# modal-labs/modal-examples

Measured on AMD Instinct MI355X. Metric: SDXL 1024px images/sec (whole node), higher is better.
Workload: dtype bf16; 1 GPU; model=sdxl-base-unet-2.6b, global_batch=16, image=1024x1024, denoise_steps=4, parallelism=dp1, hipgraph=True

## Files before the change

modal_examples_amd/models/sdxl/layers.py:

```python
from __future__ import annotations

import math

import torch
import torch.nn as nn

from ...ops import functional as OF


class _F32ParamCache:

    def _f32(self, name: str):
        p = getattr(self, name)
        if self.training or p.requires_grad and torch.is_grad_enabled():
            return p.float()
        cache = self.__dict__.setdefault("_f32_cache", {})
        ent = cache.get(name)
        if ent is None or ent[1] is not p or ent[2] != p._version:
            ent = (p.detach().float(), p, p._version)
            cache[name] = ent
        return ent[0]


class LayerNormK(nn.Module, _F32ParamCache):

    def __init__(self, dim: int, eps: float = 1e-5):
        super().__init__()
        self.weight = nn.Parameter(torch.ones(dim))
        self.bias = nn.Parameter(torch.zeros(dim))
        self.eps = eps

    def forward(self, x):
        return OF.layernorm(x, self._f32("weight"), self._f32("bias"), self.eps)


class RMSNormK(nn.Module, _F32ParamCache):
    def __init__(self, dim: int, eps: float = 1e-6):
        super().__init__()
        self.weight = nn.Parameter(torch.ones(dim))
        self.eps = eps

    def forward(self, x):
        return OF.rmsnorm(x, self._f32("weight"), self.eps)


class GroupNormSiLU(nn.Module, _F32ParamCache):

    def __init__(self, channels: int, groups: int = 32, eps: float = 1e-5,
                 silu: bool = True):
        super().__init__()
        self.weight = nn.Parameter(torch.ones(channels))
        self.bias = nn.Parameter(torch.zeros(channels))
        self.groups = groups
        self.eps = eps
        self.silu = silu

    def forward(self, x):
        return OF.groupnorm_silu(x, self._f32("weight"), self._f32("bias"),
                                 self.groups, self.eps, self.silu)


class Conv3x3(nn.Conv2d):

    def __init__(self, c_in: int, c_out: int):
        super().__init__(c_in, c_out, 3, padding=1)

    def _packed(self):
        w, bias = self.weight, self.bias
        bv = None if bias is None else bias._version
        ent = self.__dict__.get("_wr_cache")
        if (ent is None or ent[1] is not w or ent[2] != w._version
                or ent[3] is not bias or ent[4] != bv):
            wr = OF.repack_conv3x3_weight(w.detach())
            b = (bias.detach().float().contiguous() if bias is not None
                 else torch.zeros(w.shape[0], device=w.device))
            ent = ((wr, b), w, w._version, bias, bv)
            self.__dict__["_wr_cache"] = ent
        return ent[0]

    def _use_kernel(self, x) -> bool:
        if not x.is_cuda or x.dtype is not torch.bfloat16 or self.training:
            return False
        if torch.is_grad_enabled() and (x.requires_grad or
                                        self.weight.requires_grad):
            return False
        return True

    def forward_gn(self, x, gn, residual=None, upsample: bool = False):
        if self._use_kernel(x) and gn.silu:
            wr, b = self._packed()
            return OF.conv3x3_gn(x, wr, b, self.out_channels,
                                 gn._f32("weight"), gn._f32("bias"),
                                 gn.groups, gn.eps, residual=residual,
                                 raw_weight=self.weight, upsample=upsample)
        return self.forward(gn(x), residual=residual, upsample=upsample)

    def forward(self, x, residual=None, upsample: bool = False):
        if self._use_kernel(x):
            wr, b = self._packed()
            return OF.conv3x3(x, wr, b, self.out_channels, residual=residual,
                              raw_weight=self.weight, upsample=upsample)
        if upsample:
            x = nn.functional.interpolate(x, scale_factor=2.0, mode="nearest")
        y = nn.functional.conv2d(x, self.weight, self.bias, padding=1)
        return y if residual is None else y + residual


class Conv1x1(nn.Conv2d):

    def __init__(self, c_in: int, c_out: int):
        super().__init__(c_in, c_out, 1)


class SelfAttention(nn.Module):

    def __init__(self, dim: int, head_dim: int = 64):
        super().__init__()
        assert dim % head_dim == 0
        self.heads = dim // head_dim
        self.head_dim = head_dim
        self.qkv = nn.Linear(dim, 3 * dim, bias=False)
        self.out = nn.Linear(dim, dim, bias=True)

    def forward(self, x):
        B, S, C = x.shape
        qkv = self.qkv(x).view(B, S, 3, self.heads, self.head_dim)
        o = OF.attention_qkv(qkv[:, :, 0], qkv[:, :, 1], qkv[:, :, 2])
        return self.out(o)


class CrossAttention(nn.Module):

    def __init__(self, dim: int, ctx_dim: int, head_dim: int = 64):
        super().__init__()
        self.heads = dim // head_dim
        self.head_dim = head_dim
        self.q = nn.Linear(dim, dim, bias=False)
        self.kv = nn.Linear(ctx_dim, 2 * dim, bias=False)
        self.out = nn.Linear(dim, dim, bias=True)

    def forward(self, x, ctx):
        B, S, C = x.shape
        Sk = ctx.shape[1]
        q = self.q(x).view(B, S, self.heads, self.head_dim)
        kv = self.kv(ctx).view(B, Sk, 2, self.heads, self.head_dim)
        o = OF.attention_qkv(q, kv[:, :, 0], kv[:, :, 1])
        return self.out(o)


class GEGLUFeedForward(nn.Module):

    def __init__(self, dim: int, mult: int = 4):
        super().__init__()
        inner = dim * mult
        self.proj_in = nn.Linear(dim, 2 * inner, bias=True)
        self.proj_out = nn.Linear(inner, dim, bias=True)
        self.inner = inner

    def forward(self, x):
        return self.proj_out(OF.glu_fused(self.proj_in(x), gelu=True))


class TransformerBlock(nn.Module):

    def __init__(self, dim: int, ctx_dim: int, head_dim: int = 64):
        super().__init__()
        self.norm1 = LayerNormK(dim)
        self.attn1 = SelfAttention(dim, head_dim)
        self.norm2 = LayerNormK(dim)
        self.attn2 = CrossAttention(dim, ctx_dim, head_dim)
        self.norm3 = LayerNormK(dim)
        self.ff = GEGLUFeedForward(dim)

    def forward(self, x, ctx):
        x = x + self.attn1(self.norm1(x))
        x = x + self.attn2(self.norm2(x), ctx)
        x = x + self.ff(self.norm3(x))
        return x


def timestep_embedding(t: torch.Tensor, dim: int, max_period: float = 10000.0):
    half = dim // 2
    freqs = torch.exp(
        -math.log(max_period) * torch.arange(half, dtype=torch.float32, device=t.device) / half
    )
    args = t.float()[:, None] * freqs[None]
    return torch.cat([torch.cos(args), torch.sin(args)], dim=-1)
```

modal_examples_amd/models/sdxl/unet.py:

```python
from __future__ import annotations

from dataclasses import dataclass

import torch
import torch.nn as nn

from .layers import (
    Conv1x1,
    Conv3x3,
    GroupNormSiLU,
    TransformerBlock,
    timestep_embedding,
)


@dataclass
class UNetConfig:
    in_channels: int = 4
    out_channels: int = 4
    channels: tuple = (320, 640, 1280)
    layers_per_block: int = 2
    transformer_depth: tuple = (0, 2, 10)
    ctx_dim: int = 2048
    head_dim: int = 64
    time_embed_dim: int = 1280
    pooled_dim: int = 1280
    fourier_dim: int = 128
    addition_dim: int = 2816

    @staticmethod
    def sdxl() -> "UNetConfig":
        return UNetConfig()

    @staticmethod
    def small() -> "UNetConfig":
        return UNetConfig(channels=(64, 128, 256), transformer_depth=(0, 1, 2),
                          ctx_dim=256, head_dim=64, time_embed_dim=256,
                          pooled_dim=256, fourier_dim=16,
                          addition_dim=256 + 6 * 32)


class ResnetBlock(nn.Module):
    def __init__(self, c_in: int, c_out: int, temb_dim: int):
        super().__init__()
        self.norm1 = GroupNormSiLU(c_in)
        self.conv1 = Conv3x3(c_in, c_out)
        self.temb_proj = nn.Linear(temb_dim, c_out)
        self.norm2 = GroupNormSiLU(c_out)
        self.conv2 = Conv3x3(c_out, c_out)
        self.skip = Conv1x1(c_in, c_out) if c_in != c_out else nn.Identity()

    def forward(self, x, temb):
        h = self.conv1(self.norm1(x))
        h = h + self.temb_proj(torch.nn.functional.silu(temb))[:, :, None, None]
        return self.conv2(self.norm2(h), residual=self.skip(x))


class SpatialTransformer(nn.Module):

    def __init__(self, channels: int, depth: int, ctx_dim: int, head_dim: int):
        super().__init__()
        self.norm = GroupNormSiLU(channels, silu=False)
        self.proj_in = nn.Linear(channels, channels)
        self.blocks = nn.ModuleList(
            [TransformerBlock(channels, ctx_dim, head_dim) for _ in range(depth)]
        )
        self.proj_out = nn.Linear(channels, channels)

    def forward(self, x, ctx):
        B, C, H, W = x.shape
        res = x
        h = self.norm(x).permute(0, 2, 3, 1).reshape(B, H * W, C)
        h = self.proj_in(h)
        for blk in self.blocks:
            h = blk(h, ctx)
        h = self.proj_out(h)
        return res + h.reshape(B, H, W, C).permute(0, 3, 1, 2)


class Downsample(nn.Module):
    def __init__(self, c):
        super().__init__()
        self.conv = nn.Conv2d(c, c, 3, stride=2, padding=1)

    def forward(self, x):
        return self.conv(x)


class Upsample(nn.Module):
    def __init__(self, c):
        super().__init__()
        self.conv = Conv3x3(c, c)

    def forward(self, x):
        return self.conv(x, upsample=True)


class UNetXL(nn.Module):
    def __init__(self, cfg: UNetConfig = None):
        super().__init__()
        cfg = cfg or UNetConfig.sdxl()
        self.cfg = cfg
        ch = cfg.channels
        ted = cfg.time_embed_dim

        self.conv_in = Conv3x3(cfg.in_channels, ch[0])
        self.time_mlp = nn.Sequential(
            nn.Linear(ch[0], ted), nn.SiLU(), nn.Linear(ted, ted)
        )
        self.add_mlp = nn.Sequential(
            nn.Linear(cfg.addition_dim, ted), nn.SiLU(), nn.Linear(ted, ted)
        )

        self.down_blocks = nn.ModuleList()
        self.downsamplers = nn.ModuleList()
        skip_chs = [ch[0]]
        c_prev = ch[0]
        for lvl, c in enumerate(ch):
            blocks = nn.ModuleList()
            for _ in range(cfg.layers_per_block):
                entry = nn.ModuleDict({"resnet": ResnetBlock(c_prev, c, ted)})
                if cfg.transformer_depth[lvl] > 0:
                    entry["attn"] = SpatialTransformer(
                        c, cfg.transformer_depth[lvl], cfg.ctx_dim, cfg.head_dim
                    )
                blocks.append(entry)
                c_prev = c
                skip_chs.append(c)
            self.down_blocks.append(blocks)
            if lvl < len(ch) - 1:
                self.downsamplers.append(Downsample(c))
                skip_chs.append(c)
            else:
                self.downsamplers.append(nn.Identity())

        top = ch[-1]
        self.mid_res1 = ResnetBlock(top, top, ted)
        self.mid_attn = SpatialTransformer(top, cfg.transformer_depth[-1],
                                           cfg.ctx_dim, cfg.head_dim)
        self.mid_res2 = ResnetBlock(top, top, ted)

        self.up_blocks = nn.ModuleList()
        self.upsamplers = nn.ModuleList()
        c_prev = top
        for lvl in reversed(range(len(ch))):
            c = ch[lvl]
            blocks = nn.ModuleList()
            for _ in range(cfg.layers_per_block + 1):
                skip_c = skip_chs.pop()
                entry = nn.ModuleDict(
                    {"resnet": ResnetBlock(c_prev + skip_c, c, ted)}
                )
                if cfg.transformer_depth[lvl] > 0:
                    entry["attn"] = SpatialTransformer(
                        c, cfg.transformer_depth[lvl], cfg.ctx_dim, cfg.head_dim
                    )
                blocks.append(entry)
                c_prev = c
            self.up_blocks.append(blocks)
            if lvl > 0:
                self.upsamplers.append(Upsample(c))
            else:
                self.upsamplers.append(nn.Identity())

        self.norm_out = GroupNormSiLU(ch[0])
        self.conv_out = Conv3x3(ch[0], cfg.out_channels)

    def forward(self, x, t, ctx, pooled_add):
        dt = x.dtype
        temb = self.time_mlp(timestep_embedding(t, self.cfg.channels[0]).to(dt))
        temb = temb + self.add_mlp(pooled_add)

        h = self.conv_in(x)
        skips = [h]
        for lvl, blocks in enumerate(self.down_blocks):
            for entry in blocks:
                h = entry["resnet"](h, temb)
                if "attn" in entry:
                    h = entry["attn"](h, ctx)
                skips.append(h)
            if not isinstance(self.downsamplers[lvl], nn.Identity):
                h = self.downsamplers[lvl](h)
                skips.append(h)

        h = self.mid_res1(h, temb)
        h = self.mid_attn(h, ctx)
        h = self.mid_res2(h, temb)

        for i, blocks in enumerate(self.up_blocks):
            for entry in blocks:
                h = torch.cat([h, skips.pop()], dim=1)
                h = entry["resnet"](h, temb)
                if "attn" in entry:
                    h = entry["attn"](h, ctx)
            if not isinstance(self.upsamplers[i], nn.Identity):
                h = self.upsamplers[i](h)

        return self.conv_out(self.norm_out(h))
```

modal_examples_amd/models/sdxl/vae.py:

```python
from __future__ import annotations

import torch
import torch.nn as nn

from .layers import Conv1x1, Conv3x3, GroupNormSiLU


class VAEResnet(nn.Module):
    def __init__(self, c_in, c_out):
        super().__init__()
        self.norm1 = GroupNormSiLU(c_in)
        self.conv1 = Conv3x3(c_in, c_out)
        self.norm2 = GroupNormSiLU(c_out)
        self.conv2 = Conv3x3(c_out, c_out)
        self.skip = Conv1x1(c_in, c_out) if c_in != c_out else nn.Identity()

    def forward(self, x):
        h = self.conv1(self.norm1(x))
        return self.conv2(self.norm2(h), residual=self.skip(x))


class VAEMidAttention(nn.Module):

    def __init__(self, c, chunk=2048):
        super().__init__()
        self.norm = GroupNormSiLU(c, silu=False)
        self.q = nn.Linear(c, c)
        self.k = nn.Linear(c, c)
        self.v = nn.Linear(c, c)
        self.out = nn.Linear(c, c)
        self.chunk = chunk
        self.scale = c ** -0.5

    def forward(self, x):
        B, C, H, W = x.shape
        h = self.norm(x).permute(0, 2, 3, 1).reshape(B, H * W, C)
        q, k, v = self.q(h), self.k(h), self.v(h)
        outs = []
        for i in range(0, q.shape[1], self.chunk):
            s = torch.matmul(q[:, i:i + self.chunk], k.transpose(1, 2)) * self.scale
            p = torch.softmax(s.float(), dim=-1).to(v.dtype)
            outs.append(torch.matmul(p, v))
        o = self.out(torch.cat(outs, dim=1))
        return x + o.reshape(B, H, W, C).permute(0, 3, 1, 2)


class VAEDecoder(nn.Module):
    def __init__(self, latent_channels=4, channels=(512, 512, 256, 128),
                 out_channels=3, resnets_per_level=3, scaling_factor=0.13025):
        super().__init__()
        self.scaling_factor = scaling_factor
        c0 = channels[0]
        self.conv_in = Conv3x3(latent_channels, c0)
        self.mid_res1 = VAEResnet(c0, c0)
        self.mid_attn = VAEMidAttention(c0)
        self.mid_res2 = VAEResnet(c0, c0)
        self.levels = nn.ModuleList()
        c_prev = c0
        for li, c in enumerate(channels):
            blocks = nn.ModuleList()
            for _ in range(resnets_per_level):
                blocks.append(VAEResnet(c_prev, c))
                c_prev = c
            up = Conv3x3(c, c) if li < len(channels) - 1 else None
            self.levels.append(nn.ModuleList([blocks, nn.ModuleList([up] if up else [])]))
        self.norm_out = GroupNormSiLU(channels[-1])
        self.conv_out = Conv3x3(channels[-1], out_channels)

    def forward(self, z):
        h = self.conv_in(z / self.scaling_factor)
        h = self.mid_res2(self.mid_attn(self.mid_res1(h)))
        for blocks, ups in self.levels:
            for blk in blocks:
                h = blk(h)
            if len(ups):
                h = ups[0](h, upsample=True)
        return self.conv_out(self.norm_out(h))


class VAEDecoderSmall(VAEDecoder):
    def __init__(self):
        super().__init__(channels=(64, 64, 32, 32))
```

modal_examples_amd/ops/csrc/bindings.cpp:

```cpp
#include <torch/extension.h>
#include <c10/hip/HIPStream.h>
#include <hip/hip_runtime.h>

#include <unordered_map>
#include <vector>

extern "C" {
int fa32_fwd_strided_bf16(const void*, const void*, const void*, void*, float*,
                          int, int, int, int, int, int, float, int,
                          const long long*, hipStream_t);
int fa_bwd_strided_bf16(const void*, const void*, const void*, const void*,
                        const void*, const float*, float*, void*, void*, void*,
                        int, int, int, int, int, int, float, int,
                        const long long*, hipStream_t);
int paged_decode_bf16(const void*, const void*, const void*, const int*,
                      const int*, void*, float*, int, int, int, int, int,
                      int, int, float, int, hipStream_t);
int paged_prefill_bf16(const void*, const void*, const void*, const int*,
                       const int*, const int*, void*, int, int, int, int, int,
                       int, int, float, int, hipStream_t);
void groupnorm_silu_bf16(const void*, void*, float*, const float*,
                         const float*, int, int, long long, int, float, int,
                         hipStream_t);
void layernorm_bf16(const void*, void*, const float*, const float*, long long,
                    int, float, hipStream_t);
void rmsnorm_bf16(const void*, void*, const float*, long long, int, float,
                  hipStream_t);
void cfg_euler_bf16(const void*, const void*, const void*, void*, float, float,
                    long long, hipStream_t);
void silu_mul_bf16(const void*, const void*, void*, long long, hipStream_t);
void geglu_bf16(const void*, const void*, void*, long long, hipStream_t);
void glu_fused_bf16(const void*, void*, long long, long long, int,
                    hipStream_t);
void add_bf16(const void*, const void*, void*, long long, hipStream_t);
void rope_bf16(void*, const float*, const float*, long long, int, int, int,
               long long, long long, long long, const int*, hipStream_t);
void adamw_step(void*, const void*, float*, float*, long long, float, float,
                float, float, float, int, int, hipStream_t);
void gumbel_sample(const float*, unsigned long long*, int*, int, int,
                   float, unsigned long long, hipStream_t);
void sampling_cutoff(const float*, const float*, const int*, const float*,
                     const float*, float*, int, int, hipStream_t);
void gumbel_sample_batch(const float*, const float*, const long long*,
                         const long long*, const float*, unsigned long long*,
                         int*, int, int, hipStream_t);
void softmax_rows(const float*, float*, int, int, hipStream_t);
void scale_in_dev_bf16(const void*, void*, const float*, const long long*,
                       long long, hipStream_t);
void cfg_euler_dev_bf16(const void*, const void*, const void*, void*,
                        const float*, const long long*, float, long long,
                        hipStream_t);
void advance_step(long long*, hipStream_t);
void conv3x3_bf16(const void*, const void*, const void*, const void*, void*,
                  const float*, const float*, int, int, int, int, int, int,
                  int, int, hipStream_t);
void gn_conv_coeffs_bf16(const void*, float*, const float*, const float*,
                         float*, float*, int, int, int, long long, int, float,
                         hipStream_t);
int moe_max_tiles(long long, int, int);
int moe_route_f32(const float*, float*, int*, long long, int, int,
                  hipStream_t);
int moe_ffn_bf16(const void*, const void*, const void*, const float*,
                 const int*, int*, void*, float*, void*, long long, int, int,
                 int, int, hipStream_t);
}

namespace {

hipStream_t cur_stream() {
  return (hipStream_t)c10::hip::getCurrentHIPStream().stream();
}

void check_bf16(const torch::Tensor& t, const char* name) {
  TORCH_CHECK(t.is_cuda(), name, " must be on GPU");
  TORCH_CHECK(t.scalar_type() == torch::kBFloat16, name, " must be bf16");
  TORCH_CHECK(t.is_contiguous(), name, " must be contiguous");
}


void check_bhsd(const torch::Tensor& t, const char* name) {
  TORCH_CHECK(t.is_cuda(), name, " must be on GPU");
  TORCH_CHECK(t.scalar_type() == torch::kBFloat16, name, " must be bf16");
  TORCH_CHECK(t.dim() == 4, name, " must be [B,H,S,D]");
  TORCH_CHECK(t.stride(3) == 1, name, ": head_dim must be contiguous");
}

struct AttnDims {
  int B, Hq, Hkv, Sq, Sk, D;
};

AttnDims check_qkv(const char* op, const torch::Tensor& q,
                   const torch::Tensor& k, const torch::Tensor& v) {
  check_bhsd(q, "q");
  check_bhsd(k, "k");
  check_bhsd(v, "v");
  AttnDims d{(int)q.size(0), (int)q.size(1), (int)k.size(1), (int)q.size(2),
             (int)k.size(2), (int)q.size(3)};
  TORCH_CHECK(d.D == 64 || d.D == 128, op, ": unsupported head_dim ", d.D,
              " (supported: 64, 128)");
  TORCH_CHECK(k.size(0) == d.B && k.size(3) == d.D && v.sizes() == k.sizes(),
              op, ": k/v must be [B,Hkv,Sk,D] matching q's B and D");
  TORCH_CHECK(d.Hkv > 0 && d.Hq % d.Hkv == 0,
              "GQA requires Hq % Hkv == 0, got Hq=", d.Hq, " Hkv=", d.Hkv);
  return d;
}

void push_strides(std::vector<long long>& st, const torch::Tensor& t) {
  st.insert(st.end(), {t.stride(0), t.stride(1), t.stride(2)});
}

std::tuple<torch::Tensor, torch::Tensor> attention_fwd(
    const torch::Tensor& q, const torch::Tensor& k, const torch::Tensor& v,
    bool causal, double scale, bool bshd, bool with_lse,
    const c10::optional<torch::Tensor>& out = c10::nullopt,
    const c10::optional<torch::Tensor>& lse_out = c10::nullopt) {
  const AttnDims d = check_qkv("attention", q, k, v);
  TORCH_CHECK(d.Sk >= 1, "attention: Sk must be at least 1, got Sk=", d.Sk,
              " (a query with no key has no softmax)");
  const std::vector<int64_t> o_shape =
      bshd ? std::vector<int64_t>{d.B, d.Sq, d.Hq, d.D}
           : std::vector<int64_t>{d.B, d.Hq, d.Sq, d.D};
  torch::Tensor o;
  if (out.has_value()) {
    o = *out;
    TORCH_CHECK(o.device() == q.device() && o.scalar_type() == torch::kBFloat16 &&
                o.sizes() == torch::IntArrayRef(o_shape) &&
                (o.numel() == 0 || o.stride(3) == 1),
                "attention: out must be bf16 on the GPU with the output's "
                "shape ", torch::IntArrayRef(o_shape), " and head_dim "
                "contiguous");
  } else {
    o = torch::empty(o_shape, q.options());
  }
  torch::Tensor lse;
  if (with_lse) {
    if (lse_out.has_value()) {
      lse = *lse_out;
      TORCH_CHECK(lse.device() == q.device() && lse.scalar_type() == torch::kFloat32 &&
                  lse.dim() == 3 && lse.size(0) == d.B &&
                  lse.size(1) == d.Hq && lse.size(2) == d.Sq &&
                  lse.is_contiguous(),
                  "attention: lse must be fp32 [B,Hq,Sq] contiguous");
    } else {
      lse = torch::empty({d.B, d.Hq, d.Sq},
                         q.options().dtype(torch::kFloat32));
    }
  }
  if (o.numel() == 0) return {o, lse};
  std::vector<long long> st;
  for (const auto& t : {q, k, v, bshd ? o.transpose(1, 2) : o})
    push_strides(st, t);
  int rc = fa32_fwd_strided_bf16(
      q.data_ptr(), k.data_ptr(), v.data_ptr(), o.data_ptr(),
      with_lse ? lse.data_ptr<float>() : nullptr, d.B, d.Hq, d.Hkv, d.Sq,
      d.Sk, d.D, (float)scale, causal ? 1 : 0, st.data(), cur_stream());
  TORCH_CHECK(rc == 0, "attention: configuration not supported by the kernel "
              "(head_dim must be 64 or 128 and Hq a multiple of Hkv; got D=",
              d.D, " Hq=", d.Hq, " Hkv=", d.Hkv, ")");
  return {o, lse};
}

torch::Tensor attention(torch::Tensor q, torch::Tensor k, torch::Tensor v,
                        bool causal, double scale) {
  check_bf16(q, "q");
  check_bf16(k, "k");
  check_bf16(v, "v");
  return std::get<0>(attention_fwd(q, k, v, causal, scale, false, false));
}

torch::Tensor attention_bshd(torch::Tensor q, torch::Tensor k, torch::Tensor v,
                             bool causal, double scale) {
  return std::get<0>(attention_fwd(q, k, v, causal, scale, true, false));
}

std::tuple<torch::Tensor, torch::Tensor> attention_fwd_lse(
    torch::Tensor q, torch::Tensor k, torch::Tensor v, bool causal,
    double scale, c10::optional<torch::Tensor> out,
    c10::optional<torch::Tensor> lse) {
  return attention_fwd(q, k, v, causal, scale, false, true, out, lse);
}

std::tuple<torch::Tensor, torch::Tensor> attention_fwd_lse_bshd(
    torch::Tensor q, torch::Tensor k, torch::Tensor v, bool causal,
    double scale, c10::optional<torch::Tensor> out,
    c10::optional<torch::Tensor> lse) {
  return attention_fwd(q, k, v, causal, scale, true, true, out, lse);
}

torch::Tensor paged_decode(torch::Tensor q, torch::Tensor kc, torch::Tensor vc,
                           c10::optional<torch::Tensor> block_table,
                           torch::Tensor seq_lens, int64_t block_size,
                           double scale) {
  check_bf16(q, "q");
  const bool kv_fp8 = kc.scalar_type() == torch::kFloat8_e4m3fn;
  TORCH_CHECK(kv_fp8 || kc.scalar_type() == torch::kBFloat16,
              "k_cache must be bf16 or float8_e4m3fn");
  TORCH_CHECK(vc.scalar_type() == kc.scalar_type(), "kv cache dtype mismatch");
  TORCH_CHECK(kc.is_contiguous() && vc.is_contiguous());
  TORCH_CHECK(q.dim() == 3 && kc.dim() == 4, "q must be [B,Hq,D], k_cache "
              "[blocks,Hkv,block_size,D] or [B,Hkv,S,D]");
  int B = q.size(0), Hq = q.size(1), D = q.size(2);
  int Hkv = kc.size(1), max_blocks = 0;
  TORCH_CHECK(D == 64 || D == 128, "paged_decode: unsupported head_dim ", D,
              " (supported: 64, 128)");
  TORCH_CHECK(kc.size(3) == D, "paged_decode: k_cache head_dim ", kc.size(3),
              " != q head_dim ", D);
  TORCH_CHECK(Hkv > 0 && Hq % Hkv == 0, "GQA requires Hq % Hkv == 0, got Hq=",
              Hq, " Hkv=", Hkv);
  TORCH_CHECK(Hq / Hkv <= 8, "paged_decode: unsupported GQA group Hq/Hkv = ",
              Hq / Hkv, " (supported: 1..8)");
  const int* bt_ptr = nullptr;
  if (block_table.has_value()) {
    max_blocks = block_table->size(1);
    bt_ptr = block_table->data_ptr<int>();
  } else {
    block_size = kc.size(2);
  }
  auto o = torch::empty_like(q);
  long long s_bound = block_table.has_value()
      ? (long long)max_blocks * block_size : (long long)kc.size(2);
  int splits = 1;
  while (B * Hkv * splits < 512 && (long long)splits * 128 < s_bound &&
         splits < 64)
    splits *= 2;
  torch::Tensor ws;
  float* ws_ptr = nullptr;
  if (splits > 1) {
    ws = torch::empty({(long long)B * Hq * splits * (D + 2)},
                      q.options().dtype(torch::kFloat32));
    ws_ptr = ws.data_ptr<float>();
  }
  int rc = paged_decode_bf16(q.data_ptr(), kc.data_ptr(), vc.data_ptr(),
                             bt_ptr, seq_lens.data_ptr<int>(), o.data_ptr(),
                             ws_ptr, B, Hq, Hkv, D, (int)block_size,
                             max_blocks, splits, (float)scale, kv_fp8 ? 1 : 0,
                             cur_stream());
  TORCH_CHECK(rc == 0, "paged_decode: configuration not supported by the "
              "kernel (head_dim must be 64 or 128, Hq a multiple of Hkv and "
              "Hq/Hkv in 1..8; got D=", D, " Hq=", Hq, " Hkv=", Hkv, ")");
  return o;
}

torch::Tensor paged_prefill(torch::Tensor q, torch::Tensor kc, torch::Tensor vc,
                            torch::Tensor block_table, torch::Tensor cu_q,
                            torch::Tensor seq_lens, int64_t block_size,
                            double scale, int64_t max_q_len) {
  check_bf16(q, "q");
  TORCH_CHECK(q.dim() == 3, "paged_prefill: q must be [T,Hq,D]");
  const bool kv_fp8 = kc.scalar_type() == torch::kFloat8_e4m3fn;
  TORCH_CHECK(kv_fp8 || kc.scalar_type() == torch::kBFloat16,
              "k_cache must be bf16 or float8_e4m3fn");
  TORCH_CHECK(vc.scalar_type() == kc.scalar_type(), "kv cache dtype mismatch");
  TORCH_CHECK(kc.dim() == 4 && vc.sizes() == kc.sizes() &&
                  kc.is_contiguous() && vc.is_contiguous(),
              "paged_prefill: k_cache/v_cache must be contiguous "
              "[blocks,Hkv,block_size,D] of one shape");
  const int64_t T = q.size(0);
  const int Hq = q.size(1), D = q.size(2), Hkv = kc.size(1);
  TORCH_CHECK(D == 64 || D == 128, "paged_prefill: unsupported head_dim ", D,
              " (supported: 64, 128)");
  TORCH_CHECK(kc.size(3) == D, "paged_prefill: k_cache head_dim ", kc.size(3),
              " != q head_dim ", D);
  TORCH_CHECK(Hkv > 0 && Hq % Hkv == 0, "GQA requires Hq % Hkv == 0, got Hq=",
              Hq, " Hkv=", Hkv);
  TORCH_CHECK(block_size > 0 && kc.size(2) == block_size,
              "paged_prefill: block_size must be positive and the cache's "
              "third dim, got block_size=", block_size, " cache ", kc.sizes());
  TORCH_CHECK(seq_lens.scalar_type() == torch::kInt32 && seq_lens.dim() == 1 &&
                  seq_lens.is_contiguous(),
              "paged_prefill: seq_lens must be int32 [B] contiguous");
  const int64_t B = seq_lens.size(0);
  TORCH_CHECK(block_table.scalar_type() == torch::kInt32 &&
                  block_table.dim() == 2 && block_table.size(0) == B &&
                  block_table.is_contiguous(),
              "paged_prefill: block_table must be int32 [B=", B,
              ", max_blocks] contiguous, got ", block_table.sizes());
  TORCH_CHECK(cu_q.scalar_type() == torch::kInt32 && cu_q.dim() == 1 &&
                  cu_q.size(0) == B + 1 && cu_q.is_contiguous(),
              "paged_prefill: cu_q must be int32 [B+1=", B + 1, "], got ",
              cu_q.sizes());
  for (const torch::Tensor* t : {&kc, &vc, &block_table, &cu_q, &seq_lens})
    TORCH_CHECK(t->device() == q.device(),
                "paged_prefill: all tensors must be on q's device");
  auto o = torch::empty_like(q);
  if (T == 0) return o;
  TORCH_CHECK(max_q_len >= 1, "paged_prefill: max_q_len must be at least 1, "
              "got ", max_q_len);
  TORCH_CHECK(B >= 1, "paged_prefill: ", T, " query rows but no sequence");
  max_q_len = std::min<int64_t>(max_q_len, T);
  int rc = paged_prefill_bf16(
      q.data_ptr(), kc.data_ptr(), vc.data_ptr(), block_table.data_ptr<int>(),
      cu_q.data_ptr<int>(), seq_lens.data_ptr<int>(), o.data_ptr(), (int)B, Hq,
      Hkv, D, (int)block_size, (int)block_table.size(1), (int)max_q_len,
      (float)scale, kv_fp8 ? 1 : 0, cur_stream());
  TORCH_CHECK(rc == 0, "paged_prefill: configuration not supported by the "
              "kernel (head_dim must be 64 or 128, Hq a multiple of Hkv, B "
              "and Hq at most 65535; got D=", D, " Hq=", Hq, " Hkv=", Hkv,
              " B=", B, ")");
  return o;
}

void attention_bwd(torch::Tensor q, torch::Tensor k, torch::Tensor v,
                   torch::Tensor o, torch::Tensor lse, torch::Tensor dout,
                   torch::Tensor dq, torch::Tensor dk, torch::Tensor dv,
                   bool causal, double scale) {
  const AttnDims d = check_qkv("attention_bwd", q, k, v);
  const int B = d.B, Hq = d.Hq, Hkv = d.Hkv, Sq = d.Sq, Sk = d.Sk, D = d.D;
  check_bhsd(o, "o");
  check_bhsd(dout, "dout");
  check_bhsd(dq, "dq");
  check_bhsd(dk, "dk");
  check_bhsd(dv, "dv");
  TORCH_CHECK(B >= 1 && Sq >= 1 && Sk >= 1, "attention_bwd: empty input");
  TORCH_CHECK(o.sizes() == q.sizes() && dout.sizes() == q.sizes(),
              "attention_bwd: o and dout must have q's shape");
  TORCH_CHECK(dq.sizes() == q.sizes() && dk.sizes() == k.sizes() &&
              dv.sizes() == v.sizes(),
              "attention_bwd: dq/dk/dv must have the shapes of q/k/v");
  TORCH_CHECK(lse.is_cuda() && lse.scalar_type() == torch::kFloat32 &&
              lse.dim() == 3 && lse.size(0) == B && lse.size(1) == Hq &&
              lse.size(2) == Sq && lse.is_contiguous(),
              "attention_bwd: lse must be fp32 [B,Hq,Sq] contiguous");
  TORCH_CHECK(!causal || Sk >= Sq, "attention_bwd: causal requires Sk >= Sq, "
              "got Sq=", Sq, " Sk=", Sk);
  auto delta = torch::empty_like(lse);
  std::vector<long long> st;
  for (const auto& t : {q, k, v, o, dout, dq, dk, dv}) push_strides(st, t);
  int rc = fa_bwd_strided_bf16(
      q.data_ptr(), k.data_ptr(), v.data_ptr(), o.data_ptr(), dout.data_ptr(),
      lse.data_ptr<float>(), delta.data_ptr<float>(), dq.data_ptr(),
      dk.data_ptr(), dv.data_ptr(), B, Hq, Hkv, Sq, Sk, D, (float)scale,
      causal ? 1 : 0, st.data(), cur_stream());
  TORCH_CHECK(rc == 0, "attention_bwd: configuration not supported by the "
              "kernel (got D=", D, " Hq=", Hq, " Hkv=", Hkv, " Sq=", Sq,
              " Sk=", Sk, " causal=", causal, ")");
}


torch::Tensor groupnorm_silu(torch::Tensor x, torch::Tensor gamma,
                             torch::Tensor beta, int64_t groups, double eps,
                             bool do_silu) {
  check_bf16(x, "x");
  TORCH_CHECK(x.dim() == 4, "x must be NCHW");
  int N = x.size(0), C = x.size(1);
  long long HW = (long long)x.size(2) * x.size(3);
  auto y = torch::empty_like(x);
  auto ws = torch::zeros({N * groups * 2},
                         x.options().dtype(torch::kFloat32));
  groupnorm_silu_bf16(x.data_ptr(), y.data_ptr(), ws.data_ptr<float>(),
                      gamma.data_ptr<float>(), beta.data_ptr<float>(), N, C,
                      HW, (int)groups, (float)eps, do_silu ? 1 : 0,
                      cur_stream());
  return y;
}

torch::Tensor layernorm(torch::Tensor x, torch::Tensor gamma,
                        torch::Tensor beta, double eps) {
  check_bf16(x, "x");
  int D = x.size(-1);
  long long rows = x.numel() / D;
  auto y = torch::empty_like(x);
  layernorm_bf16(x.data_ptr(), y.data_ptr(), gamma.data_ptr<float>(),
                 beta.data_ptr<float>(), rows, D, (float)eps, cur_stream());
  return y;
}

torch::Tensor rmsnorm(torch::Tensor x, torch::Tensor gamma, double eps) {
  check_bf16(x, "x");
  int D = x.size(-1);
  TORCH_CHECK(D % 8 == 0, "rmsnorm needs D % 8 == 0");
  long long rows = x.numel() / D;
  auto y = torch::empty_like(x);
  rmsnorm_bf16(x.data_ptr(), y.data_ptr(), gamma.data_ptr<float>(), rows, D,
               (float)eps, cur_stream());
  return y;
}


torch::Tensor cfg_euler(torch::Tensor xt, torch::Tensor eps_c,
                        c10::optional<torch::Tensor> eps_u, double guidance,
                        double dsigma) {
  check_bf16(xt, "x_t");
  auto xn = torch::empty_like(xt);
  cfg_euler_bf16(xt.data_ptr(), eps_c.data_ptr(),
                 eps_u.has_value() ? eps_u->data_ptr() : nullptr,
                 xn.data_ptr(), (float)guidance, (float)dsigma, xt.numel(),
                 cur_stream());
  return xn;
}

torch::Tensor silu_mul(torch::Tensor a, torch::Tensor b) {
  check_bf16(a, "a");
  auto y = torch::empty_like(a);
  silu_mul_bf16(a.data_ptr(), b.data_ptr(), y.data_ptr(), a.numel(),
                cur_stream());
  return y;
}

torch::Tensor geglu(torch::Tensor a, torch::Tensor b) {
  check_bf16(a, "a");
  auto y = torch::empty_like(a);
  geglu_bf16(a.data_ptr(), b.data_ptr(), y.data_ptr(), a.numel(), cur_stream());
  return y;
}

torch::Tensor glu_fused(torch::Tensor src, bool gelu) {
  check_bf16(src, "src");
  long long inner = src.size(-1) / 2;
  TORCH_CHECK(src.size(-1) % 2 == 0 && inner % 8 == 0,
              "inner dim must be even and 8-aligned");
  long long rows = src.numel() / (2 * inner);
  auto sizes = src.sizes().vec();
  sizes.back() = inner;
  auto y = torch::empty(sizes, src.options());
  glu_fused_bf16(src.data_ptr(), y.data_ptr(), rows, inner, gelu ? 1 : 0,
                 cur_stream());
  return y;
}

torch::Tensor add_residual(torch::Tensor a, torch::Tensor b) {
  check_bf16(a, "a");
  auto y = torch::empty_like(a);
  add_bf16(a.data_ptr(), b.data_ptr(), y.data_ptr(), a.numel(), cur_stream());
  return y;
}

void rope_(torch::Tensor qk, torch::Tensor cosv, torch::Tensor sinv,
           c10::optional<torch::Tensor> positions) {
  TORCH_CHECK(qk.is_cuda() && qk.scalar_type() == torch::kBFloat16);
  TORCH_CHECK(qk.dim() == 4 && qk.stride(3) == 1,
              "qk must be [B,H,S,D] with contiguous head_dim");
  long long B = qk.size(0);
  int H = qk.size(1), S = qk.size(2), D = qk.size(3);
  if (positions.has_value())
    TORCH_CHECK(positions->numel() == B * S || positions->numel() == S,
                "positions must be [B*S] (or [S] with B==1)");
  rope_bf16(qk.data_ptr(), cosv.data_ptr<float>(), sinv.data_ptr<float>(), B,
            H, S, D, qk.stride(0), qk.stride(1), qk.stride(2),
            positions.has_value() ? positions->data_ptr<int>() : nullptr,
            cur_stream());
}

void adamw_(torch::Tensor p, torch::Tensor g, torch::Tensor m, torch::Tensor v,
            double lr, double beta1, double beta2, double eps, double wd,
            int64_t step) {
  TORCH_CHECK(p.is_cuda() && p.is_contiguous(), "p must be contiguous GPU");
  bool bf16 = p.scalar_type() == torch::kBFloat16;
  adamw_step(p.data_ptr(), g.data_ptr(), m.data_ptr<float>(),
             v.data_ptr<float>(), p.numel(), (float)lr, (float)beta1,
             (float)beta2, (float)eps, (float)wd, (int)step, bf16 ? 1 : 0,
             cur_stream());
}


void check_f32_vec(const torch::Tensor& t, const char* name, int64_t n,
                   const char* len) {
  TORCH_CHECK(t.is_cuda(), name, " must be on GPU");
  TORCH_CHECK(t.scalar_type() == torch::kFloat, name, " must be fp32");
  TORCH_CHECK(t.is_contiguous(), name, " must be contiguous");
  TORCH_CHECK(t.numel() == n, name, " must have ", len, " = ", n,
              " elements, got ", t.numel());
}

struct ConvDims {
  int N, C, H, W, Ho, Wo, Kpad, C16;
};

ConvDims check_conv(const char* op, const torch::Tensor& x,
                    const torch::Tensor& wr, const torch::Tensor& bias,
                    const c10::optional<torch::Tensor>& residual, int64_t K,
                    bool upsample) {
  check_bf16(x, "x");
  check_bf16(wr, "wr");
  TORCH_CHECK(x.dim() == 4, op, ": x must be NCHW, got ", x.dim(), " dims");
  TORCH_CHECK(wr.dim() == 3 && wr.size(0) == 9 && wr.size(1) > 0 &&
                  wr.size(2) > 0 && wr.size(1) % 64 == 0 &&
                  wr.size(2) % 16 == 0,
              op, ": wr must be [9, Kpad, C16] (repacked 3x3 weights) with "
              "Kpad % 64 == 0 and C16 % 16 == 0, got ", wr.sizes());
  ConvDims d{(int)x.size(0), (int)x.size(1), (int)x.size(2), (int)x.size(3),
             0, 0, (int)wr.size(1), (int)wr.size(2)};
  d.Ho = upsample ? d.H * 2 : d.H;
  d.Wo = upsample ? d.W * 2 : d.W;
  TORCH_CHECK(K >= 1, op, ": K must be at least 1, got ", K);
  TORCH_CHECK(K <= d.Kpad && d.C <= d.C16, op,
              ": weight pack smaller than conv (K=", K, " > Kpad=", d.Kpad,
              " or C=", d.C, " > C16=", d.C16, ")");
  TORCH_CHECK((int64_t)d.C16 * d.H * d.W < (1ll << 30) &&
                  64ll * d.Ho * d.Wo < (1ll << 31) &&
                  9ll * d.Kpad * d.C16 < (1ll << 31),
              op, ": too large for the kernel's 32-bit offsets (C16*H*W must "
              "stay below 2^30, 64*Ho*Wo and 9*Kpad*C16 below 2^31), got x ",
              x.sizes(), " wr ", wr.sizes());
  check_f32_vec(bias, "bias", K, "K");
  if (residual.has_value()) {
    check_bf16(*residual, "residual");
    TORCH_CHECK(residual->dim() == 4 && residual->size(0) == d.N &&
                    residual->size(1) == K && residual->size(2) == d.Ho &&
                    residual->size(3) == d.Wo,
                op, ": residual shape mismatch: ", residual->sizes(),
                " against output [", d.N, ", ", K, ", ", d.Ho, ", ", d.Wo, "]");
  }
  return d;
}

torch::Tensor conv3x3(torch::Tensor x, torch::Tensor wr, torch::Tensor bias,
                      c10::optional<torch::Tensor> residual, int64_t K,
                      bool upsample) {
  const ConvDims d = check_conv("conv3x3", x, wr, bias, residual, K, upsample);
  auto out = torch::empty({d.N, K, d.Ho, d.Wo}, x.options());
  conv3x3_bf16(x.data_ptr(), wr.data_ptr(), bias.data_ptr(),
               residual.has_value() ? residual->data_ptr() : nullptr,
               out.data_ptr(), nullptr, nullptr, d.N, d.C, d.Ho, d.Wo, (int)K,
               d.C16, d.Kpad, upsample ? 1 : 0, cur_stream());
  return out;
}

torch::Tensor conv3x3_gn(torch::Tensor x, torch::Tensor wr, torch::Tensor bias,
                         c10::optional<torch::Tensor> residual, int64_t K,
                         bool upsample, torch::Tensor gamma,
                         torch::Tensor beta, int64_t groups, double eps) {
  const ConvDims d =
      check_conv("conv3x3_gn", x, wr, bias, residual, K, upsample);
  check_f32_vec(gamma, "gamma", d.C, "C");
  check_f32_vec(beta, "beta", d.C, "C");
  TORCH_CHECK(groups >= 1 && d.C % groups == 0,
              "conv3x3_gn: groups must be at least 1 and divide C, got groups=",
              groups, " C=", d.C);
  const int N = d.N, C16 = d.C16;
  long long HW = (long long)d.H * d.W;
  auto fopt = x.options().dtype(torch::kFloat32);
  auto ws = torch::zeros({(long long)N * groups * 2}, fopt);
  auto scale = torch::empty({(long long)N * C16}, fopt);
  auto shift = torch::empty({(long long)N * C16}, fopt);
  gn_conv_coeffs_bf16(x.data_ptr(), ws.data_ptr<float>(),
                      gamma.data_ptr<float>(), beta.data_ptr<float>(),
                      scale.data_ptr<float>(), shift.data_ptr<float>(), N, d.C,
                      C16, HW, (int)groups, (float)eps, cur_stream());
  auto out = torch::empty({N, K, d.Ho, d.Wo}, x.options());
  conv3x3_bf16(x.data_ptr(), wr.data_ptr(), bias.data_ptr(),
               residual.has_value() ? residual->data_ptr() : nullptr,
               out.data_ptr(), scale.data_ptr<float>(),
               shift.data_ptr<float>(), N, d.C, d.Ho, d.Wo, (int)K, C16,
               d.Kpad, upsample ? 1 : 0, cur_stream());
  return out;
}


std::tuple<torch::Tensor, torch::Tensor> moe_route(torch::Tensor logits,
                                                   int64_t top_k) {
  TORCH_CHECK(logits.is_cuda() && logits.scalar_type() == torch::kFloat32 &&
                  logits.dim() == 2 && logits.is_contiguous(),
              "moe_route: logits must be fp32 [N,E] contiguous on GPU");
  const int64_t N = logits.size(0), E = logits.size(1);
  TORCH_CHECK(N >= 1, "moe_route: logits has no rows");
  TORCH_CHECK(E >= 1 && E <= 128, "moe_route: logits has E=", E,
              " experts (supported: 1..128)");
  TORCH_CHECK(top_k >= 1 && top_k <= 8 && top_k <= E, "moe_route: top_k=",
              top_k, " (supported: 1..min(E, 8), E=", E, ")");
  auto w = torch::empty({N, top_k}, logits.options());
  auto idx = torch::empty({N, top_k}, logits.options().dtype(torch::kInt32));
  int rc = moe_route_f32(logits.data_ptr<float>(), w.data_ptr<float>(),
                         idx.data_ptr<int>(), N, (int)E, (int)top_k,
                         cur_stream());
  TORCH_CHECK(rc == 0, "moe_route: logits shape ", logits.sizes(),
              " with top_k=", top_k, " not supported by the kernel");
  return {w, idx};
}

torch::Tensor moe_ffn(torch::Tensor x, torch::Tensor gate_up,
                      torch::Tensor down, torch::Tensor weights,
                      torch::Tensor idx) {
  check_bf16(x, "x");
  check_bf16(gate_up, "gate_up");
  check_bf16(down, "down");
  TORCH_CHECK(x.dim() == 2 && gate_up.dim() == 3 && down.dim() == 3,
              "moe_ffn: x must be [N,dim], gate_up [E,2*ffn_dim,dim], down "
              "[E,dim,ffn_dim]");
  const int64_t N = x.size(0), d = x.size(1), E = gate_up.size(0),
                F = down.size(2);
  TORCH_CHECK(N >= 1, "moe_ffn: x has no rows");
  TORCH_CHECK(d >= 64 && d % 64 == 0, "moe_ffn: x has dim=", d,
              " (must be a multiple of 64)");
  TORCH_CHECK(F >= 64 && F % 64 == 0, "moe_ffn: down has ffn_dim=", F,
              " (must be a multiple of 64)");
  TORCH_CHECK(E >= 1 && E <= 128, "moe_ffn: gate_up has E=", E,
              " experts (supported: 1..128)");
  TORCH_CHECK(gate_up.size(1) == 2 * F && gate_up.size(2) == d &&
                  down.size(0) == E && down.size(1) == d,
              "moe_ffn: gate_up ", gate_up.sizes(), " / down ", down.sizes(),
              " do not match [E,2*ffn_dim,dim] / [E,dim,ffn_dim] with dim=",
              d);
  TORCH_CHECK(idx.is_cuda() && idx.scalar_type() == torch::kInt32 &&
                  idx.dim() == 2 && idx.size(0) == N && idx.is_contiguous(),
              "moe_ffn: idx must be int32 [N,top_k] contiguous on GPU");
  const int64_t k = idx.size(1);
  TORCH_CHECK(k >= 1 && k <= 8 && k <= E, "moe_ffn: idx has top_k=", k,
              " (supported: 1..min(E, 8), E=", E, ")");
  TORCH_CHECK(weights.is_cuda() && weights.scalar_type() == torch::kFloat32 &&
                  weights.sizes() == idx.sizes() && weights.is_contiguous(),
              "moe_ffn: weights must be fp32 [N,top_k] contiguous on GPU");
  for (const torch::Tensor* t : {&gate_up, &down, &weights, &idx})
    TORCH_CHECK(t->device() == x.device(),
                "moe_ffn: all tensors must be on x's device");
  TORCH_CHECK(N * k < (1ll << 30) && N * k * d < (1ll << 40),
              "moe_ffn: x has too many rows (N=", N, ")");
  const int64_t tiles = moe_max_tiles(N, (int)k, (int)E);
  auto iopt = x.options().dtype(torch::kInt32);
  auto sched = torch::empty({tiles * 32 + tiles + 1}, iopt);
  auto h = torch::empty({tiles * 32, F}, x.options());
  auto y = torch::empty({N * k, d}, x.options().dtype(torch::kFloat32));
  auto out = torch::empty({N, d}, x.options());
  int rc = moe_ffn_bf16(x.data_ptr(), gate_up.data_ptr(), down.data_ptr(),
                        weights.data_ptr<float>(), idx.data_ptr<int>(),
                        sched.data_ptr<int>(), h.data_ptr(),
                        y.data_ptr<float>(), out.data_ptr(), N, (int)d,
                        (int)F, (int)E, (int)k, cur_stream());
  TORCH_CHECK(rc == 0, "moe_ffn: shape not supported by the kernel (N=", N,
              " dim=", d, " ffn_dim=", F, " E=", E, " top_k=", k, ")");
  return out;
}

torch::Tensor sample_gumbel(torch::Tensor logits, double temperature,
                            int64_t seed) {
  TORCH_CHECK(logits.is_cuda() && logits.scalar_type() == torch::kFloat32,
              "logits must be f32 GPU");
  int rows = logits.size(0), V = logits.size(1);
  auto out = torch::empty({rows}, logits.options().dtype(torch::kInt32));
  auto keys = torch::zeros({rows}, logits.options().dtype(torch::kInt64));
  gumbel_sample(logits.data_ptr<float>(),
                (unsigned long long*)keys.data_ptr<int64_t>(),
                out.data_ptr<int>(), rows, V, (float)temperature,
                (unsigned long long)seed, cur_stream());
  return out;
}


void check_logits2d(const torch::Tensor& logits) {
  TORCH_CHECK(logits.is_cuda() && logits.scalar_type() == torch::kFloat32,
              "logits must be f32 GPU");
  TORCH_CHECK(logits.dim() == 2 && logits.is_contiguous(),
              "logits must be [rows, V] contiguous");
  TORCH_CHECK(logits.size(0) > 0 && logits.size(1) > 0 &&
              logits.size(1) < (1ll << 31) && logits.size(0) < (1ll << 22),
              "logits: unsupported shape ", logits.sizes());
}

void check_row_param(const torch::Tensor& t, const torch::Tensor& logits,
                     torch::ScalarType dt, const char* name) {
  TORCH_CHECK(t.is_cuda() && t.device() == logits.device(), name,
              " must be on the logits' GPU");
  TORCH_CHECK(t.scalar_type() == dt, name, " must be ", dt);
  TORCH_CHECK(t.dim() == 1 && t.size(0) == logits.size(0), name,
              " must have one value per row ([", logits.size(0), "]), got ",
              t.sizes());
  TORCH_CHECK(t.is_contiguous(), name, " must be contiguous");
}

torch::Tensor sampling_cutoff_fwd(torch::Tensor logits, torch::Tensor temps,
                                  torch::Tensor top_k, torch::Tensor top_p,
                                  torch::Tensor min_p) {
  check_logits2d(logits);
  check_row_param(temps, logits, torch::kFloat32, "temperature");
  check_row_param(top_k, logits, torch::kInt32, "top_k");
  check_row_param(top_p, logits, torch::kFloat32, "top_p");
  check_row_param(min_p, logits, torch::kFloat32, "min_p");
  int rows = logits.size(0), V = logits.size(1);
  auto cut = torch::empty({rows}, logits.options());
  sampling_cutoff(logits.data_ptr<float>(), temps.data_ptr<float>(),
                  top_k.data_ptr<int>(), top_p.data_ptr<float>(),
                  min_p.data_ptr<float>(), cut.data_ptr<float>(), rows, V,
                  cur_stream());
  return cut;
}

torch::Tensor sample_batch(torch::Tensor logits, torch::Tensor temps,
                           torch::Tensor seeds, torch::Tensor counters,
                           c10::optional<torch::Tensor> cutoff) {
  check_logits2d(logits);
  check_row_param(temps, logits, torch::kFloat32, "temperature");
  check_row_param(seeds, logits, torch::kInt64, "seeds");
  check_row_param(counters, logits, torch::kInt64, "counters");
  if (cutoff.has_value())
    check_row_param(*cutoff, logits, torch::kFloat32, "cutoff");
  int rows = logits.size(0), V = logits.size(1);
  auto out = torch::empty({rows}, logits.options().dtype(torch::kInt32));
  auto keys = torch::zeros({rows}, logits.options().dtype(torch::kInt64));
  gumbel_sample_batch(
      logits.data_ptr<float>(), temps.data_ptr<float>(),
      (const long long*)seeds.data_ptr<int64_t>(),
      (const long long*)counters.data_ptr<int64_t>(),
      cutoff.has_value() ? cutoff->data_ptr<float>() : nullptr,
      (unsigned long long*)keys.data_ptr<int64_t>(), out.data_ptr<int>(),
      rows, V, cur_stream());
  return out;
}

torch::Tensor softmax_fwd(torch::Tensor x) {
  TORCH_CHECK(x.is_cuda() && x.scalar_type() == torch::kFloat32);
  int V = x.size(-1);
  long long rows = x.numel() / V;
  auto y = torch::empty_like(x);
  softmax_rows(x.data_ptr<float>(), y.data_ptr<float>(), (int)rows, V,
               cur_stream());
  return y;
}

void scale_in_dev(torch::Tensor x, torch::Tensor y, torch::Tensor sigmas,
                  torch::Tensor step) {
  scale_in_dev_bf16(x.data_ptr(), y.data_ptr(), sigmas.data_ptr<float>(),
                    (const long long*)step.data_ptr<int64_t>(), x.numel(), cur_stream());
}

void cfg_euler_dev(torch::Tensor xt, torch::Tensor eps_c,
                   c10::optional<torch::Tensor> eps_u, torch::Tensor xn,
                   torch::Tensor sigmas, torch::Tensor step, double guidance) {
  cfg_euler_dev_bf16(xt.data_ptr(), eps_c.data_ptr(),
                     eps_u.has_value() ? eps_u->data_ptr() : nullptr,
                     xn.data_ptr(), sigmas.data_ptr<float>(),
                     (const long long*)step.data_ptr<int64_t>(), (float)guidance, xt.numel(),
                     cur_stream());
}

void step_advance(torch::Tensor step) {
  advance_step((long long*)step.data_ptr<int64_t>(), cur_stream());
}


struct SnapRegion {
  void* host = nullptr;
  size_t bytes = 0;
  std::vector<hipStream_t> streams;
  size_t rr = 0;
};

std::unordered_map<int64_t, SnapRegion> g_snaps;
int64_t g_next_snap = 1;

int64_t snap_create(int64_t bytes) {
  SnapRegion r;
  r.bytes = (size_t)bytes;
  TORCH_CHECK(hipHostMalloc(&r.host, r.bytes, hipHostMallocDefault) == hipSuccess,
              "hipHostMalloc failed for ", bytes, " bytes");
  r.streams.resize(4);
  for (auto& s : r.streams)
    TORCH_CHECK(hipStreamCreateWithFlags(&s, hipStreamNonBlocking) == hipSuccess);
  int64_t id = g_next_snap++;
  g_snaps[id] = r;
  return id;
}

void snap_save(int64_t id, int64_t offset, torch::Tensor t) {
  auto& r = g_snaps.at(id);
  size_t n = t.numel() * t.element_size();
  TORCH_CHECK((size_t)offset + n <= r.bytes, "snapshot overflow");
  hipStream_t s = r.streams[r.rr++ % r.streams.size()];
  TORCH_CHECK(hipMemcpyAsync((char*)r.host + offset, t.data_ptr(), n,
                             hipMemcpyDeviceToHost, s) == hipSuccess);
}

void snap_restore(int64_t id, int64_t offset, torch::Tensor t) {
  auto& r = g_snaps.at(id);
  size_t n = t.numel() * t.element_size();
  TORCH_CHECK((size_t)offset + n <= r.bytes, "snapshot overflow");
  hipStream_t s = r.streams[r.rr++ % r.streams.size()];
  TORCH_CHECK(hipMemcpyAsync(t.data_ptr(), (char*)r.host + offset, n,
                             hipMemcpyHostToDevice, s) == hipSuccess);
}

void snap_sync(int64_t id) {
  auto& r = g_snaps.at(id);
  for (auto& s : r.streams) TORCH_CHECK(hipStreamSynchronize(s) == hipSuccess);
}

void snap_free(int64_t id) {
  auto it = g_snaps.find(id);
  if (it == g_snaps.end()) return;
  for (auto& s : it->second.streams) hipStreamDestroy(s);
  hipHostFree(it->second.host);
  g_snaps.erase(it);
}

}

PYBIND11_MODULE(TORCH_EXTENSION_NAME, m) {
  m.def("attention", &attention, "flash attention fwd bf16 (K1/K5/K7)");
  m.def("attention_bshd", &attention_bshd, "stride-aware attention, BSHD out");
  m.def("attention_fwd_lse", &attention_fwd_lse,
        "attention fwd returning (o, lse) for the backward; out= / lse= "
        "write into the caller's tensors",
        py::arg("q"), py::arg("k"), py::arg("v"), py::arg("causal"),
        py::arg("scale"), py::arg("out") = py::none(),
        py::arg("lse") = py::none());
  m.def("attention_fwd_lse_bshd", &attention_fwd_lse_bshd,
        "attention fwd returning (o [B,S,H,D], lse); out= / lse= write into "
        "the caller's tensors",
        py::arg("q"), py::arg("k"), py::arg("v"), py::arg("causal"),
        py::arg("scale"), py::arg("out") = py::none(),
        py::arg("lse") = py::none());
  m.def("attention_bwd", &attention_bwd,
        "flash attention bwd bf16 into caller-provided dq/dk/dv");
  m.def("paged_decode", &paged_decode, "paged KV decode attention (K6)");
  m.def("paged_prefill", &paged_prefill,
        "paged KV prefill attention: ragged causal chunks over a cached "
        "prefix (K6)");
  m.def("groupnorm_silu", &groupnorm_silu);
  m.def("layernorm", &layernorm);
  m.def("rmsnorm", &rmsnorm);
  m.def("cfg_euler", &cfg_euler, "fused CFG + Euler step (K4)");
  m.def("silu_mul", &silu_mul);
  m.def("geglu", &geglu);
  m.def("glu_fused", &glu_fused, "in-place-sliced silu/gelu-mul over a fused [.,2I] projection");
  m.def("add_residual", &add_residual);
  m.def("rope_", &rope_, "in-place RoPE with host cos/sin tables");
  m.def("adamw_", &adamw_, "fused AdamW step (K9)");
  m.def("sample_gumbel", &sample_gumbel, "fused sampling (K8)");
  m.def("sample_batch", &sample_batch,
        "per-row temperature/seed/counter/cutoff gumbel sampling (K8)");
  m.def("sampling_cutoff", &sampling_cutoff_fwd,
        "per-row top-k/top-p/min-p logit cutoff by radix select (K8)");
  m.def("conv3x3", &conv3x3, "NCHW implicit-GEMM 3x3 conv, fused bias+res (K3)");
  m.def("conv3x3_gn", &conv3x3_gn, "GroupNorm+SiLU fused into the K3 conv");
  m.def("softmax_fwd", &softmax_fwd);
  m.def("moe_route", &moe_route,
        "MoE top-k routing: (weights fp32 [N,k], idx int32 [N,k])");
  m.def("moe_ffn", &moe_ffn,
        "fused MoE FFN: on-device schedule, grouped MFMA GEMMs, combine");
  m.def("scale_in_dev", &scale_in_dev, "x * 1/sqrt(sigma^2+1), device sigma");
  m.def("cfg_euler_dev", &cfg_euler_dev, "graph-capturable CFG+Euler step");
  m.def("step_advance", &step_advance, "increment device step counter");
  m.def("snap_create", &snap_create, "pinned-host snapshot region (K13)");
  m.def("snap_save", &snap_save);
  m.def("snap_restore", &snap_restore);
  m.def("snap_sync", &snap_sync);
  m.def("snap_free", &snap_free);
}
```

modal_examples_amd/ops/csrc/conv3x3.hip:

```cpp
#include "common.h"

#include <cstdio>
#include <cstdlib>
#include <type_traits>

#define CV_NW 4
#define CV_COLS 32
#define CV_BK 64
#define CV_CC 16

typedef __attribute__((ext_vector_type(16))) float f32x16c;

DEV_INLINE unsigned gn_silu_bf16(unsigned raw, float sc, float sh) {
  float f = bf2f((short)raw) * sc + sh;
  f = f / (1.f + __expf(-f));
  return (unsigned)(unsigned short)f2bf(f);
}

DEV_INLINE int to_sgpr(int v) {
  int s;
  asm volatile("s_nop 0\n\tv_readfirstlane_b32 %0, %1" : "=s"(s) : "v"(v));
  return s;
}

#define PATCH_C (CV_COLS + 2)

#define WLDS_ELEMS (9 * CV_BK * CV_CC)
#define WSLOTS (WLDS_ELEMS / 8)
#define WSLOTS_PER_T ((WSLOTS + CV_NW * WAVE - 1) / (CV_NW * WAVE))

template <bool UP, bool GN, int RPW>
__global__ __launch_bounds__(CV_NW * WAVE, RPW == 2 ? 3 : 1)
void conv3x3_kernel(
    const short* __restrict__ in, const short* __restrict__ wr,
    const float* __restrict__ bias, const short* __restrict__ res,
    short* __restrict__ out, const float* __restrict__ gn_scale,
    const float* __restrict__ gn_shift, int C, int H, int W, int Hs, int Ws,
    int K, int C16, int Kpad, int npix_x, int npix, int nk) {
  constexpr int CV_ROWS = CV_NW * RPW;
  constexpr int PATCH_R = CV_ROWS + 2;
  constexpr int PATCH_ELEMS = PATCH_R * PATCH_C * CV_CC;
  constexpr int STAGE_SLOTS = PATCH_R * PATCH_C * 2;
  constexpr int SLOTS_PER_T =
      (STAGE_SLOTS + CV_NW * WAVE - 1) / (CV_NW * WAVE);
  __shared__ alignas(16) short patch[PATCH_ELEMS];
  __shared__ alignas(16) short wlds[WLDS_ELEMS];
  __shared__ alignas(16) float bias_s[CV_BK];

  const int tid = threadIdx.x;
  const int w = tid / WAVE;
  const int l = tid % WAVE;
  const int l31 = l & 31;
  const int hi5 = l >> 5;
  const int n = blockIdx.y;

  int bid = blockIdx.x;
  {
    int nwg = npix * nk;
    int q = nwg >> 3, r = nwg & 7;
    int xcd = bid & 7, pos = bid >> 3;
    bid = (xcd < r ? xcd * (q + 1) : r * (q + 1) + (xcd - r) * q) + pos;
  }
  const int ktile = to_sgpr(bid / npix);
  const int pix = bid - ktile * npix;
  const int pix_y = pix / npix_x;
  const int y0 = pix_y * CV_ROWS;
  const int x0 = (pix - pix_y * npix_x) * CV_COLS;
  const int k0 = ktile * CV_BK;

  const long long in_n = (long long)n * C * Hs * Ws;
  const int nc = C16 / CV_CC;

  if (tid < CV_BK) bias_s[tid] = bias[min(k0 + tid, K - 1)];

  const char* in_img = (const char*)(in + in_n);
  const unsigned hwb = (unsigned)Hs * (unsigned)Ws * 2u;
  unsigned soff[SLOTS_PER_T], soff_max[SLOTS_PER_T];
  int slds[SLOTS_PER_T], smask[SLOTS_PER_T];
#pragma unroll
  for (int i = 0; i < SLOTS_PER_T; ++i) {
    const int s_raw = i * CV_NW * WAVE + tid;
    const int s = min(s_raw, STAGE_SLOTS - 1);
    const int col = s % PATCH_C;
    const int u = s / PATCH_C;
    const int oct = u & 1;
    const int row = u >> 1;
    const int y = y0 + row - 1;
    const int x = x0 + col - 1;
    const bool live =
        s_raw < STAGE_SLOTS && y >= 0 && y < H && x >= 0 && x < W;
    const int yc = min(max(y, 0), H - 1);
    const int xc = min(max(x, 0), W - 1);
    const unsigned sy = UP ? (yc >> 1) : yc;
    const unsigned sx = UP ? (xc >> 1) : xc;
    const unsigned pix = (sy * (unsigned)Ws + sx) * 2u;
    soff[i] = pix + (unsigned)(oct * 8) * hwb;
    soff_max[i] = pix + (unsigned)(C - 1) * hwb;
    slds[i] = (row * PATCH_C + col) * CV_CC + oct * 8;
    int m = live ? -1 : 0;
    asm volatile("" : "+v"(m));
    smask[i] = m;
  }

  unsigned sraw[SLOTS_PER_T][8];
  float gsc[GN ? CV_CC : 1], gsh[GN ? CV_CC : 1];
  auto stage_load = [&](int cc) {
#pragma unroll
    for (int i = 0; i < SLOTS_PER_T; ++i) {
#pragma unroll
      for (int j = 0; j < 8; ++j) {
        const unsigned o = min(soff[i] + (unsigned)j * hwb, soff_max[i]);
        sraw[i][j] = *(const unsigned short*)(in_img + o);
      }
      soff[i] += CV_CC * hwb;
    }
    if constexpr (GN) {
      const float* ps = gn_scale + (long long)n * C16 + cc * CV_CC;
      const float* ph = gn_shift + (long long)n * C16 + cc * CV_CC;
#pragma unroll
      for (int j = 0; j < CV_CC; ++j) {
        gsc[j] = ps[j];
        gsh[j] = ph[j];
      }
    }
  };
  auto stage_write = [&](int cc) {
    const int nv = C - cc * CV_CC;
#pragma unroll
    for (int i = 0; i < SLOTS_PER_T; ++i) {
      const int o8 = slds[i] & 8;
      i32x4 pk;
#pragma unroll
      for (int d = 0; d < 4; ++d) {
        unsigned lo = sraw[i][2 * d], hi = sraw[i][2 * d + 1];
        asm volatile("" : "+v"(lo), "+v"(hi));
        if constexpr (GN) {
          lo = gn_silu_bf16(lo, o8 ? gsc[8 + 2 * d] : gsc[2 * d],
                            o8 ? gsh[8 + 2 * d] : gsh[2 * d]);
          hi = gn_silu_bf16(hi, o8 ? gsc[9 + 2 * d] : gsc[1 + 2 * d],
                            o8 ? gsh[9 + 2 * d] : gsh[1 + 2 * d]);
        }
        pk[d] = (int)((lo | (hi << 16)) & (unsigned)smask[i]);
      }
      if (nv < CV_CC) {
        const int nvl = nv - o8;
#pragma unroll
        for (int d = 0; d < 4; ++d) {
          const unsigned lo = (unsigned)((2 * d - nvl) >> 31);
          const unsigned hi = (unsigned)((2 * d + 1 - nvl) >> 31);
          pk[d] &= (int)((lo & 0xffffu) | (hi & 0xffff0000u));
        }
      }
      if ((i + 1) * CV_NW * WAVE <= STAGE_SLOTS ||
          i * CV_NW * WAVE + tid < STAGE_SLOTS)
        *(i32x4*)&patch[slds[i]] = pk;
    }
  };

  bf16x8 wreg[WSLOTS_PER_T];
  unsigned woff[WSLOTS_PER_T];
#pragma unroll
  for (int i = 0; i < WSLOTS_PER_T; ++i) {
    const int s = min(i * CV_NW * WAVE + tid, WSLOTS - 1);
    const int oct = s & 1;
    const int kr = (s >> 1) & (CV_BK - 1);
    const int tap = (s >> 1) >> 6;
    woff[i] = ((unsigned)(tap * Kpad + kr) * (unsigned)C16 + oct * 8) * 2u;
  }
  const char* w_tile = (const char*)(wr + (long long)k0 * C16);
  auto wstage_load = [&](int cc) {
    const char* wb = w_tile + cc * (CV_CC * 2);
#pragma unroll
    for (int i = 0; i < WSLOTS_PER_T; ++i)
      wreg[i] = *(const bf16x8*)(wb + woff[i]);
  };
  auto wstage_write = [&]() {
#pragma unroll
    for (int i = 0; i < WSLOTS_PER_T; ++i) {
      const int s = i * CV_NW * WAVE + tid;
      if ((i + 1) * CV_NW * WAVE <= WSLOTS || s < WSLOTS)
        *(bf16x8*)&wlds[s * 8] = wreg[i];
    }
  };

  f32x16c acc[RPW][2];
#pragma unroll
  for (int a = 0; a < RPW; ++a)
#pragma unroll
    for (int b = 0; b < 2; ++b)
#pragma unroll
      for (int r = 0; r < 16; ++r) acc[a][b][r] = 0.f;

  stage_load(0);
  wstage_load(0);
  for (int cc = 0; cc < nc; ++cc) {
    __syncthreads();
    stage_write(cc);
    wstage_write();
    __syncthreads();
    if (cc + 1 < nc) {
      stage_load(cc + 1);
      wstage_load(cc + 1);
    }

    const short* wl = &wlds[l31 * CV_CC + hi5 * 8];
    const short* pl = &patch[(w * RPW * PATCH_C + l31) * CV_CC + hi5 * 8];
#pragma unroll
    for (int tap = 0; tap < 9; ++tap) {
      const int dy = tap / 3, dx = tap - 3 * (tap / 3);
      bf16x8 a0 = *(const bf16x8*)&wl[tap * CV_BK * CV_CC];
      bf16x8 a1 = *(const bf16x8*)&wl[(tap * CV_BK + 32) * CV_CC];
#pragma unroll
      for (int rr = 0; rr < RPW; ++rr) {
        bf16x8 b =
            *(const bf16x8*)&pl[((rr + dy) * PATCH_C + dx) * CV_CC];
        __builtin_amdgcn_s_setprio(1);
        acc[rr][0] = __builtin_amdgcn_mfma_f32_32x32x16_bf16(a0, b, acc[rr][0], 0, 0, 0);
        acc[rr][1] = __builtin_amdgcn_mfma_f32_32x32x16_bf16(a1, b, acc[rr][1], 0, 0, 0);
        __builtin_amdgcn_s_setprio(0);
      }
    }
  }

  auto epilogue = [&](auto res_c, auto edge_c) {
    constexpr bool RES = decltype(res_c)::value;
    constexpr bool EDGE = decltype(edge_c)::value;
    int t = tid;
    asm volatile("" : "+v"(t));
    const int w = t / WAVE, l31 = t & 31, hi5 = (t >> 5) & 1;
    const unsigned hw = (unsigned)H * (unsigned)W;
    const long long slab = ((long long)n * K + k0) * hw;
    const char* resb = RES ? (const char*)(res + slab) : nullptr;
    char* outb = (char*)(out + slab);
    const int x = x0 + l31;
    const int kmax = K - 1 - k0;
#pragma unroll
    for (int rr = 0; rr < RPW; ++rr) {
      const int y = y0 + w * RPW + rr;
      const bool pix_ok = !EDGE || (y < H && x < W);
      const unsigned po = EDGE ? (unsigned)min(y, H - 1) * W + min(x, W - 1)
                               : (unsigned)y * W + x;
#pragma unroll
      for (int mf = 0; mf < 2; ++mf) {
        unsigned rv[16];
        if constexpr (RES) {
#pragma unroll
          for (int r = 0; r < 16; ++r) {
            const int kl = mf * 32 + (r & 3) + 8 * (r >> 2) + 4 * hi5;
            const unsigned ke = EDGE ? min(kl, kmax) : kl;
            rv[r] = *(const unsigned short*)(resb + (po + ke * hw) * 2u);
          }
        }
#pragma unroll
        for (int q = 0; q < 4; ++q) {
          const f32x4 b4 = *(const f32x4*)&bias_s[mf * 32 + 8 * q + 4 * hi5];
#pragma unroll
          for (int j = 0; j < 4; ++j) {
            const int r = q * 4 + j;
            const int kl = mf * 32 + j + 8 * q + 4 * hi5;
            float v = acc[rr][mf][r] + b4[j];
            if constexpr (RES) v += bf2f((short)rv[r]);
            if (!EDGE || (pix_ok && kl <= kmax))
              *(short*)(outb + (po + (unsigned)kl * hw) * 2u) = f2bf(v);
          }
        }
      }
    }
  };
  const bool edge =
      y0 + CV_ROWS > H || x0 + CV_COLS > W || k0 + CV_BK > K;
  if (res != nullptr) {
    if (edge) epilogue(std::true_type{}, std::true_type{});
    else epilogue(std::true_type{}, std::false_type{});
  } else {
    if (edge) epilogue(std::false_type{}, std::true_type{});
    else epilogue(std::false_type{}, std::false_type{});
  }
}

extern "C" void conv3x3_bf16(const void* in, const void* wrepack,
                             const void* bias, const void* residual, void* out,
                             const float* gn_scale, const float* gn_shift,
                             int N, int C, int H, int W, int K, int C16,
                             int Kpad, int upsample, hipStream_t stream) {
  const int Hs = upsample ? H / 2 : H;
  const int Ws = upsample ? W / 2 : W;
  static const int rpw = [] {
    const char* e = getenv("MODAL_AMD_CONV_RPW");
    return (e && atoi(e) == 4) ? 4 : 2;
  }();
  const int rows = CV_NW * rpw;
  const int npix_x = (W + CV_COLS - 1) / CV_COLS;
  const int npix_y = (H + rows - 1) / rows;
  const int npix = npix_x * npix_y;
  const int nk = (K + CV_BK - 1) / CV_BK;
  dim3 grid(npix * nk, N);
  dim3 block(CV_NW * WAVE);
  const bool gn = gn_scale != nullptr;
#define CVL(UPV, GNV, RPWV) \
  hipLaunchKernelGGL((conv3x3_kernel<UPV, GNV, RPWV>), grid, block, 0, \
                     stream, (const short*)in, (const short*)wrepack, \
                     (const float*)bias, (const short*)residual, (short*)out, \
                     gn_scale, gn_shift, C, H, W, Hs, Ws, K, C16, Kpad, \
                     npix_x, npix, nk)
  if (rpw == 4) {
    if (upsample) {
      if (gn) CVL(true, true, 4); else CVL(true, false, 4);
    } else {
      if (gn) CVL(false, true, 4); else CVL(false, false, 4);
    }
  } else {
    if (upsample) {
      if (gn) CVL(true, true, 2); else CVL(true, false, 2);
    } else {
      if (gn) CVL(false, true, 2); else CVL(false, false, 2);
    }
  }
#undef CVL
}
```

modal_examples_amd/ops/csrc/elementwise.hip:

```cpp
#include "common.h"

#define EW_BLOCK 256


__global__ __launch_bounds__(EW_BLOCK) void cfg_euler_kernel(
    const short* __restrict__ Xt, const short* __restrict__ EpsC,
    const short* __restrict__ EpsU, short* __restrict__ Xn, float guidance,
    float dsigma, long long n) {
  long long stride = (long long)gridDim.x * EW_BLOCK * 8;
  for (long long i = ((long long)blockIdx.x * EW_BLOCK + threadIdx.x) * 8;
       i + 8 <= n; i += stride) {
    bf16x8 x = *(const bf16x8*)&Xt[i];
    bf16x8 ec = *(const bf16x8*)&EpsC[i];
    bf16x8 o;
    if (EpsU != nullptr) {
      bf16x8 eu = *(const bf16x8*)&EpsU[i];
#pragma unroll
      for (int j = 0; j < 8; ++j) {
        float e = bf2f(eu[j]) + guidance * (bf2f(ec[j]) - bf2f(eu[j]));
        o[j] = f2bf(bf2f(x[j]) + dsigma * e);
      }
    } else {
#pragma unroll
      for (int j = 0; j < 8; ++j)
        o[j] = f2bf(bf2f(x[j]) + dsigma * bf2f(ec[j]));
    }
    *(bf16x8*)&Xn[i] = o;
  }
  long long full = (n / 8) * 8;
  for (long long i = full + (long long)blockIdx.x * EW_BLOCK + threadIdx.x;
       i < n; i += (long long)gridDim.x * EW_BLOCK) {
    float e = bf2f(EpsC[i]);
    if (EpsU != nullptr) {
      float eu = bf2f(EpsU[i]);
      e = eu + guidance * (e - eu);
    }
    Xn[i] = f2bf(bf2f(Xt[i]) + dsigma * e);
  }
}

extern "C" void cfg_euler_bf16(const void* xt, const void* eps_c,
                               const void* eps_u, void* xn, float guidance,
                               float dsigma, long long n, hipStream_t stream) {
  int grid = elementwise_grid(n, EW_BLOCK);
  hipLaunchKernelGGL(cfg_euler_kernel, dim3(grid), dim3(EW_BLOCK), 0, stream,
                     (const short*)xt, (const short*)eps_c,
                     (const short*)eps_u, (short*)xn, guidance, dsigma, n);
}


__global__ __launch_bounds__(EW_BLOCK) void silu_mul_kernel(
    const short* __restrict__ A, const short* __restrict__ Bv,
    short* __restrict__ Y, long long n) {
  long long stride = (long long)gridDim.x * EW_BLOCK * 8;
  for (long long i = ((long long)blockIdx.x * EW_BLOCK + threadIdx.x) * 8;
       i + 8 <= n; i += stride) {
    bf16x8 a = *(const bf16x8*)&A[i];
    bf16x8 b = *(const bf16x8*)&Bv[i];
    bf16x8 o;
#pragma unroll
    for (int j = 0; j < 8; ++j) {
      float f = bf2f(a[j]);
      o[j] = f2bf(f / (1.f + __expf(-f)) * bf2f(b[j]));
    }
    *(bf16x8*)&Y[i] = o;
  }
  long long full = (n / 8) * 8;
  for (long long i = full + (long long)blockIdx.x * EW_BLOCK + threadIdx.x;
       i < n; i += (long long)gridDim.x * EW_BLOCK) {
    float f = bf2f(A[i]);
    Y[i] = f2bf(f / (1.f + __expf(-f)) * bf2f(Bv[i]));
  }
}

extern "C" void silu_mul_bf16(const void* a, const void* b, void* y,
                              long long n, hipStream_t stream) {
  int grid = elementwise_grid(n, EW_BLOCK);
  hipLaunchKernelGGL(silu_mul_kernel, dim3(grid), dim3(EW_BLOCK), 0, stream,
                     (const short*)a, (const short*)b, (short*)y, n);
}


__global__ __launch_bounds__(EW_BLOCK) void geglu_kernel(
    const short* __restrict__ A, const short* __restrict__ Bv,
    short* __restrict__ Y, long long n) {
  long long stride = (long long)gridDim.x * EW_BLOCK * 8;
  const float k0 = 0.7978845608028654f, k1 = 0.044715f;
  for (long long i = ((long long)blockIdx.x * EW_BLOCK + threadIdx.x) * 8;
       i + 8 <= n; i += stride) {
    bf16x8 a = *(const bf16x8*)&A[i];
    bf16x8 b = *(const bf16x8*)&Bv[i];
    bf16x8 o;
#pragma unroll
    for (int j = 0; j < 8; ++j) {
      float f = bf2f(a[j]);
      float g = 0.5f * f * (1.f + tanhf(k0 * (f + k1 * f * f * f)));
      o[j] = f2bf(g * bf2f(b[j]));
    }
    *(bf16x8*)&Y[i] = o;
  }
  long long full = (n / 8) * 8;
  for (long long i = full + (long long)blockIdx.x * EW_BLOCK + threadIdx.x;
       i < n; i += (long long)gridDim.x * EW_BLOCK) {
    float f = bf2f(A[i]);
    float g = 0.5f * f * (1.f + tanhf(k0 * (f + k1 * f * f * f)));
    Y[i] = f2bf(g * bf2f(Bv[i]));
  }
}

extern "C" void geglu_bf16(const void* a, const void* b, void* y, long long n,
                           hipStream_t stream) {
  int grid = elementwise_grid(n, EW_BLOCK);
  hipLaunchKernelGGL(geglu_kernel, dim3(grid), dim3(EW_BLOCK), 0, stream,
                     (const short*)a, (const short*)b, (short*)y, n);
}


__global__ __launch_bounds__(EW_BLOCK) void add_kernel(
    const short* __restrict__ A, const short* __restrict__ Bv,
    short* __restrict__ Y, long long n) {
  long long stride = (long long)gridDim.x * EW_BLOCK * 8;
  for (long long i = ((long long)blockIdx.x * EW_BLOCK + threadIdx.x) * 8;
       i + 8 <= n; i += stride) {
    bf16x8 a = *(const bf16x8*)&A[i];
    bf16x8 b = *(const bf16x8*)&Bv[i];
    bf16x8 o;
#pragma unroll
    for (int j = 0; j < 8; ++j) o[j] = f2bf(bf2f(a[j]) + bf2f(b[j]));
    *(bf16x8*)&Y[i] = o;
  }
  long long full = (n / 8) * 8;
  for (long long i = full + (long long)blockIdx.x * EW_BLOCK + threadIdx.x;
       i < n; i += (long long)gridDim.x * EW_BLOCK)
    Y[i] = f2bf(bf2f(A[i]) + bf2f(Bv[i]));
}

extern "C" void add_bf16(const void* a, const void* b, void* y, long long n,
                         hipStream_t stream) {
  int grid = elementwise_grid(n, EW_BLOCK);
  hipLaunchKernelGGL(add_kernel, dim3(grid), dim3(EW_BLOCK), 0, stream,
                     (const short*)a, (const short*)b, (short*)y, n);
}


__global__ __launch_bounds__(EW_BLOCK) void rope_kernel(
    short* __restrict__ Qk, const float* __restrict__ Cos,
    const float* __restrict__ Sin, long long B, int H, int S, int D,
    long long bst, long long hst, long long sst,
    const int* __restrict__ positions ) {
  long long rows = B * H * S;
  int l = threadIdx.x % WAVE;
  for (long long row = blockIdx.x * (EW_BLOCK / WAVE) + threadIdx.x / WAVE;
       row < rows; row += (long long)gridDim.x * (EW_BLOCK / WAVE)) {
    int s = (int)(row % S);
    int h = (int)((row / S) % H);
    long long b = row / ((long long)H * S);
    int pos = positions != nullptr ? positions[b * S + s] : s;
    short* x = Qk + b * bst + h * hst + s * sst;
    for (int i = l * 2; i < D / 2; i += WAVE * 2) {
      float c0 = Cos[(long long)pos * (D / 2) + i];
      float s0 = Sin[(long long)pos * (D / 2) + i];
      float c1 = Cos[(long long)pos * (D / 2) + i + 1];
      float s1 = Sin[(long long)pos * (D / 2) + i + 1];
      float x0 = bf2f(x[i]), x2 = bf2f(x[i + D / 2]);
      float x1 = bf2f(x[i + 1]), x3 = bf2f(x[i + 1 + D / 2]);
      x[i] = f2bf(x0 * c0 - x2 * s0);
      x[i + D / 2] = f2bf(x2 * c0 + x0 * s0);
      x[i + 1] = f2bf(x1 * c1 - x3 * s1);
      x[i + 1 + D / 2] = f2bf(x3 * c1 + x1 * s1);
    }
  }
}

extern "C" void rope_bf16(void* qk, const float* cosv, const float* sinv,
                          long long B, int H, int S, int D, long long bst,
                          long long hst, long long sst, const int* positions,
                          hipStream_t stream) {
  long long rows = B * (long long)H * S;
  int grid = (int)((rows + 3) / 4);
  if (grid > 4096) grid = 4096;
  hipLaunchKernelGGL(rope_kernel, dim3(grid), dim3(EW_BLOCK), 0, stream,
                     (short*)qk, cosv, sinv, B, H, S, D, bst, hst, sst,
                     positions);
}


__global__ __launch_bounds__(EW_BLOCK) void scale_in_dev_kernel(
    const short* __restrict__ X, short* __restrict__ Y,
    const float* __restrict__ sigmas, const long long* __restrict__ step,
    long long n) {
  float s = sigmas[(int)*step];
  float c = rsqrtf(s * s + 1.f);
  long long stride = (long long)gridDim.x * EW_BLOCK * 8;
  for (long long i = ((long long)blockIdx.x * EW_BLOCK + threadIdx.x) * 8;
       i + 8 <= n; i += stride) {
    bf16x8 x = *(const bf16x8*)&X[i];
    bf16x8 o;
#pragma unroll
    for (int j = 0; j < 8; ++j) o[j] = f2bf(bf2f(x[j]) * c);
    *(bf16x8*)&Y[i] = o;
  }
  long long full = (n / 8) * 8;
  for (long long i = full + (long long)blockIdx.x * EW_BLOCK + threadIdx.x;
       i < n; i += (long long)gridDim.x * EW_BLOCK)
    Y[i] = f2bf(bf2f(X[i]) * c);
}

__global__ __launch_bounds__(EW_BLOCK) void cfg_euler_dev_kernel(
    const short* __restrict__ Xt, const short* __restrict__ EpsC,
    const short* __restrict__ EpsU, short* __restrict__ Xn,
    const float* __restrict__ sigmas, const long long* __restrict__ step,
    float guidance, long long n) {
  int st = (int)*step;
  float dsigma = sigmas[st + 1] - sigmas[st];
  long long stride = (long long)gridDim.x * EW_BLOCK * 8;
  for (long long i = ((long long)blockIdx.x * EW_BLOCK + threadIdx.x) * 8;
       i + 8 <= n; i += stride) {
    bf16x8 x = *(const bf16x8*)&Xt[i];
    bf16x8 ec = *(const bf16x8*)&EpsC[i];
    bf16x8 o;
    if (EpsU != nullptr) {
      bf16x8 eu = *(const bf16x8*)&EpsU[i];
#pragma unroll
      for (int j = 0; j < 8; ++j) {
        float e = bf2f(eu[j]) + guidance * (bf2f(ec[j]) - bf2f(eu[j]));
        o[j] = f2bf(bf2f(x[j]) + dsigma * e);
      }
    } else {
#pragma unroll
      for (int j = 0; j < 8; ++j)
        o[j] = f2bf(bf2f(x[j]) + dsigma * bf2f(ec[j]));
    }
    *(bf16x8*)&Xn[i] = o;
  }
  long long full = (n / 8) * 8;
  for (long long i = full + (long long)blockIdx.x * EW_BLOCK + threadIdx.x;
       i < n; i += (long long)gridDim.x * EW_BLOCK) {
    float e = bf2f(EpsC[i]);
    if (EpsU != nullptr) {
      float eu = bf2f(EpsU[i]);
      e = eu + guidance * (e - eu);
    }
    Xn[i] = f2bf(bf2f(Xt[i]) + dsigma * e);
  }
}

__global__ void advance_step_kernel(long long* step) {
  if (threadIdx.x == 0 && blockIdx.x == 0) *step += 1;
}

extern "C" void scale_in_dev_bf16(const void* x, void* y, const float* sigmas,
                                  const long long* step, long long n,
                                  hipStream_t stream) {
  int grid = elementwise_grid(n, EW_BLOCK);
  hipLaunchKernelGGL(scale_in_dev_kernel, dim3(grid), dim3(EW_BLOCK), 0,
                     stream, (const short*)x, (short*)y, sigmas, step, n);
}

extern "C" void cfg_euler_dev_bf16(const void* xt, const void* eps_c,
                                   const void* eps_u, void* xn,
                                   const float* sigmas, const long long* step,
                                   float guidance, long long n,
                                   hipStream_t stream) {
  int grid = elementwise_grid(n, EW_BLOCK);
  hipLaunchKernelGGL(cfg_euler_dev_kernel, dim3(grid), dim3(EW_BLOCK), 0,
                     stream, (const short*)xt, (const short*)eps_c,
                     (const short*)eps_u, (short*)xn, sigmas, step, guidance,
                     n);
}

extern "C" void advance_step(long long* step, hipStream_t stream) {
  hipLaunchKernelGGL(advance_step_kernel, dim3(1), dim3(64), 0, stream, step);
}


template <bool GELU>
__global__ __launch_bounds__(EW_BLOCK) void glu_fused_kernel(
    const short* __restrict__ Src, short* __restrict__ Y, long long rows,
    long long inner) {
  const float k0 = 0.7978845608028654f, k1 = 0.044715f;
  long long n = rows * inner;
  long long stride = (long long)gridDim.x * EW_BLOCK * 8;
  for (long long i = ((long long)blockIdx.x * EW_BLOCK + threadIdx.x) * 8;
       i + 8 <= n; i += stride) {
    long long row = i / inner, c = i - row * inner;
    const short* base = Src + row * 2 * inner + c;
    bf16x8 a = *(const bf16x8*)base;
    bf16x8 b = *(const bf16x8*)(base + inner);
    bf16x8 o;
#pragma unroll
    for (int j = 0; j < 8; ++j) {
      float f = bf2f(a[j]);
      float act;
      if (GELU) {
        float t = tanhf(k0 * (f + k1 * f * f * f));
        act = 0.5f * f * (1.f + t);
      } else {
        act = f / (1.f + __expf(-f));
      }
      o[j] = f2bf(act * bf2f(b[j]));
    }
    *(bf16x8*)&Y[i] = o;
  }
  long long full = (n / 8) * 8;
  for (long long i = full + (long long)blockIdx.x * EW_BLOCK + threadIdx.x;
       i < n; i += (long long)gridDim.x * EW_BLOCK) {
    long long row = i / inner, c = i - row * inner;
    float f = bf2f(Src[row * 2 * inner + c]);
    float bb = bf2f(Src[row * 2 * inner + inner + c]);
    float act;
    if (GELU) {
      float t = tanhf(k0 * (f + k1 * f * f * f));
      act = 0.5f * f * (1.f + t);
    } else {
      act = f / (1.f + __expf(-f));
    }
    Y[i] = f2bf(act * bb);
  }
}

extern "C" void glu_fused_bf16(const void* src, void* y, long long rows,
                               long long inner, int gelu,
                               hipStream_t stream) {
  int grid = elementwise_grid(rows * inner, EW_BLOCK);
  if (gelu)
    hipLaunchKernelGGL((glu_fused_kernel<true>), dim3(grid), dim3(EW_BLOCK),
                       0, stream, (const short*)src, (short*)y, rows, inner);
  else
    hipLaunchKernelGGL((glu_fused_kernel<false>), dim3(grid), dim3(EW_BLOCK),
                       0, stream, (const short*)src, (short*)y, rows, inner);
}
```

modal_examples_amd/ops/csrc/norms.hip:

```cpp
#include "common.h"


__global__ __launch_bounds__(256) void gn_partial_kernel(
    const short* __restrict__ X, float* __restrict__ WS, int N, int C,
    long long HW, int G, int split) {
  const int blk = blockIdx.x;
  const int ng = blk / split;
  const int sp = blk % split;
  const int n = ng / G, g = ng % G;
  const int cpg = C / G;
  const short* x = X + ((long long)n * C + (long long)g * cpg) * HW;
  long long per = (((HW + split - 1) / split) + 7) & ~7LL;
  long long lo = sp * per, hi = min(HW, lo + per);
  if (lo >= HW) return;
  float s = 0.f, ss = 0.f;
  for (int c = 0; c < cpg; ++c) {
    const short* xc = x + (long long)c * HW;
    long long i = lo + (long long)threadIdx.x * 8;
    for (; i + 8 <= hi; i += 256 * 8) {
      bf16x8 v = *(const bf16x8*)&xc[i];
#pragma unroll
      for (int j = 0; j < 8; ++j) {
        float f = bf2f(v[j]);
        s += f;
        ss += f * f;
      }
    }
    long long tail = hi - ((hi - lo) % 8);
    for (long long t = tail + threadIdx.x; t < hi; t += 256) {
      if (t >= lo) {
        float f = bf2f(xc[t]);
        s += f;
        ss += f * f;
      }
    }
  }
  s = wave_sum(s);
  ss = wave_sum(ss);
  if ((threadIdx.x & (WAVE - 1)) == 0) {
    atomicAdd(&WS[ng * 2], s);
    atomicAdd(&WS[ng * 2 + 1], ss);
  }
}

__global__ __launch_bounds__(256) void gn_norm_kernel(
    const short* __restrict__ X, short* __restrict__ Y,
    const float* __restrict__ WS, const float* __restrict__ gamma,
    const float* __restrict__ beta, int N, int C, long long HW, int G,
    float eps, int do_silu, int split) {
  const int blk = blockIdx.x;
  const int ng = blk / split;
  const int sp = blk % split;
  const int n = ng / G, g = ng % G;
  const int cpg = C / G;
  const long long slab = (long long)cpg * HW;
  const short* x = X + ((long long)n * C + (long long)g * cpg) * HW;
  short* y = Y + ((long long)n * C + (long long)g * cpg) * HW;
  float mean = WS[ng * 2] / (float)slab;
  float var = WS[ng * 2 + 1] / (float)slab - mean * mean;
  float rstd = rsqrtf(var + eps);
  long long per = (((HW + split - 1) / split) + 7) & ~7LL;
  long long lo = sp * per, hi = min(HW, lo + per);
  if (lo >= HW) return;
  for (int c = 0; c < cpg; ++c) {
    const short* xc = x + (long long)c * HW;
    short* yc = y + (long long)c * HW;
    float gam = gamma[g * cpg + c] * rstd;
    float bet = beta[g * cpg + c] - mean * gam;
    long long i = lo + (long long)threadIdx.x * 8;
    for (; i + 8 <= hi; i += 256 * 8) {
      bf16x8 v = *(const bf16x8*)&xc[i];
      bf16x8 o;
#pragma unroll
      for (int j = 0; j < 8; ++j) {
        float f = bf2f(v[j]) * gam + bet;
        if (do_silu) f = f / (1.f + __expf(-f));
        o[j] = f2bf(f);
      }
      *(bf16x8*)&yc[i] = o;
    }
    long long tail = hi - ((hi - lo) % 8);
    for (long long t = tail + threadIdx.x; t < hi; t += 256) {
      if (t >= lo) {
        float f = bf2f(xc[t]) * gam + bet;
        if (do_silu) f = f / (1.f + __expf(-f));
        yc[t] = f2bf(f);
      }
    }
  }
}

extern "C" void groupnorm_silu_bf16(const void* x, void* y, float* ws,
                                    const float* gamma, const float* beta,
                                    int N, int C, long long HW, int G,
                                    float eps, int do_silu,
                                    hipStream_t stream) {
  int split = 1;
  while (N * G * split < 1024 && (long long)split * 2048 < HW) split *= 2;
  dim3 grid(N * G * split);
  hipLaunchKernelGGL(gn_partial_kernel, grid, dim3(256), 0, stream,
                     (const short*)x, ws, N, C, HW, G, split);
  hipLaunchKernelGGL(gn_norm_kernel, grid, dim3(256), 0, stream,
                     (const short*)x, (short*)y, ws, gamma, beta, N, C, HW, G,
                     eps, do_silu, split);
}


__global__ __launch_bounds__(256) void layernorm_kernel(
    const short* __restrict__ X, short* __restrict__ Y,
    const float* __restrict__ gamma, const float* __restrict__ beta,
    long long rows, int D, float eps) {
  int w = threadIdx.x / WAVE, l = threadIdx.x % WAVE;
  long long row = (long long)blockIdx.x * 4 + w;
  if (row >= rows) return;
  const short* x = X + row * D;
  short* y = Y + row * D;
  float s = 0.f, ss = 0.f;
  for (int i = l * 8; i + 8 <= D; i += WAVE * 8) {
    bf16x8 v = *(const bf16x8*)&x[i];
#pragma unroll
    for (int j = 0; j < 8; ++j) {
      float f = bf2f(v[j]);
      s += f;
      ss += f * f;
    }
  }
  for (int i = (D / 8) * 8 + l; i < D; i += WAVE) {
    float f = bf2f(x[i]);
    s += f;
    ss += f * f;
  }
  s = wave_sum(s);
  ss = wave_sum(ss);
  float mean = s / D, var = ss / D - mean * mean;
  float rstd = rsqrtf(var + eps);
  for (int i = l * 8; i + 8 <= D; i += WAVE * 8) {
    bf16x8 v = *(const bf16x8*)&x[i];
    bf16x8 o;
#pragma unroll
    for (int j = 0; j < 8; ++j)
      o[j] = f2bf((bf2f(v[j]) - mean) * rstd * gamma[i + j] + beta[i + j]);
    *(bf16x8*)&y[i] = o;
  }
  for (int i = (D / 8) * 8 + l; i < D; i += WAVE)
    y[i] = f2bf((bf2f(x[i]) - mean) * rstd * gamma[i] + beta[i]);
}

extern "C" void layernorm_bf16(const void* x, void* y, const float* gamma,
                               const float* beta, long long rows, int D,
                               float eps, hipStream_t stream) {
  long long blocks = (rows + 3) / 4;
  hipLaunchKernelGGL(layernorm_kernel, dim3((unsigned)blocks), dim3(256), 0,
                     stream, (const short*)x, (short*)y, gamma, beta, rows, D,
                     eps);
}


__global__ __launch_bounds__(256) void rmsnorm_kernel(
    const short* __restrict__ X, short* __restrict__ Y,
    const float* __restrict__ gamma, long long rows, int D, float eps) {
  int w = threadIdx.x / WAVE, l = threadIdx.x % WAVE;
  long long row = (long long)blockIdx.x * 4 + w;
  if (row >= rows) return;
  const short* x = X + row * D;
  short* y = Y + row * D;
  float ss = 0.f;
  for (int i = l * 8; i + 8 <= D; i += WAVE * 8) {
    bf16x8 v = *(const bf16x8*)&x[i];
#pragma unroll
    for (int j = 0; j < 8; ++j) {
      float f = bf2f(v[j]);
      ss += f * f;
    }
  }
  ss = wave_sum(ss);
  float rstd = rsqrtf(ss / D + eps);
  for (int i = l * 8; i + 8 <= D; i += WAVE * 8) {
    bf16x8 v = *(const bf16x8*)&x[i];
    bf16x8 o;
#pragma unroll
    for (int j = 0; j < 8; ++j) o[j] = f2bf(bf2f(v[j]) * rstd * gamma[i + j]);
    *(bf16x8*)&y[i] = o;
  }
}

extern "C" void rmsnorm_bf16(const void* x, void* y, const float* gamma,
                             long long rows, int D, float eps,
                             hipStream_t stream) {
  long long blocks = (rows + 3) / 4;
  hipLaunchKernelGGL(rmsnorm_kernel, dim3((unsigned)blocks), dim3(256), 0,
                     stream, (const short*)x, (short*)y, gamma, rows, D, eps);
}



__global__ __launch_bounds__(256) void gn_coeff_kernel(
    const float* __restrict__ WS, const float* __restrict__ gamma,
    const float* __restrict__ beta, float* __restrict__ scale,
    float* __restrict__ shift, int N, int C, int Cpad, long long HW, int G,
    float eps) {
  int i = blockIdx.x * 256 + threadIdx.x;
  if (i >= N * Cpad) return;
  int n = i / Cpad, c = i % Cpad;
  if (c >= C) {
    scale[i] = 0.f;
    shift[i] = 0.f;
    return;
  }
  int cpg = C / G, g = c / cpg;
  long long slab = (long long)cpg * HW;
  float mean = WS[(n * G + g) * 2] / (float)slab;
  float var = WS[(n * G + g) * 2 + 1] / (float)slab - mean * mean;
  float rstd = rsqrtf(var + eps);
  float sc = gamma[c] * rstd;
  scale[i] = sc;
  shift[i] = beta[c] - mean * sc;
}

extern "C" void gn_conv_coeffs_bf16(const void* x, float* ws,
                                    const float* gamma, const float* beta,
                                    float* scale, float* shift, int N, int C,
                                    int Cpad, long long HW, int G, float eps,
                                    hipStream_t stream) {
  int split = 1;
  while (N * G * split < 1024 && (long long)split * 2048 < HW) split *= 2;
  hipLaunchKernelGGL(gn_partial_kernel, dim3(N * G * split), dim3(256), 0,
                     stream, (const short*)x, ws, N, C, HW, G, split);
  hipLaunchKernelGGL(gn_coeff_kernel, dim3((N * Cpad + 255) / 256), dim3(256),
                     0, stream, ws, gamma, beta, scale, shift, N, C, Cpad, HW,
                     G, eps);
}
```

modal_examples_amd/ops/csrc/sampling.hip:

```cpp
#include "common.h"

#define SMP_BLOCK 256

DEV_INLINE unsigned int hash3(unsigned int a, unsigned int b, unsigned int c) {
  unsigned int h = a * 0x9E3779B1u ^ b * 0x85EBCA77u ^ c * 0xC2B2AE3Du;
  h ^= h >> 15;
  h *= 0x2C1B3C6Du;
  h ^= h >> 12;
  h *= 0x297A2D39u;
  h ^= h >> 15;
  return h;
}

__global__ __launch_bounds__(SMP_BLOCK) void gumbel_sample_kernel(
    const float* __restrict__ Logits,
    unsigned long long* __restrict__ Keys,
    int rows, int V, int splits, float inv_temp, unsigned long long seed,
    int greedy) {
  int row = blockIdx.x / splits;
  int split = blockIdx.x % splits;
  if (row >= rows) return;
  const float* lg = Logits + (long long)row * V;
  int chunk = (V + splits - 1) / splits;
  int lo = split * chunk, hi = min(V, lo + chunk);
  float best = -1e30f;
  int best_i = lo;
  for (int i = lo + threadIdx.x; i < hi; i += SMP_BLOCK) {
    float s = lg[i] * inv_temp;
    if (!greedy) {
      unsigned int u = hash3((unsigned int)seed, (unsigned int)(seed >> 32) ^ row, i);
      float uf = (u >> 8) * (1.f / 16777216.f) + 1e-10f;
      s += -__logf(-__logf(uf));
    }
    if (s > best || (s == best && i < best_i)) {
      best = s;
      best_i = i;
    }
  }
#pragma unroll
  for (int s_ = 1; s_ < WAVE; s_ <<= 1) {
    float ov = __shfl_xor(best, s_, WAVE);
    int oi = __shfl_xor(best_i, s_, WAVE);
    if (ov > best || (ov == best && oi < best_i)) {
      best = ov;
      best_i = oi;
    }
  }
  __shared__ float sv[SMP_BLOCK / WAVE];
  __shared__ int si[SMP_BLOCK / WAVE];
  int w = threadIdx.x / WAVE;
  if (threadIdx.x % WAVE == 0) {
    sv[w] = best;
    si[w] = best_i;
  }
  __syncthreads();
  if (threadIdx.x == 0) {
    for (int j = 1; j < SMP_BLOCK / WAVE; ++j)
      if (sv[j] > best || (sv[j] == best && si[j] < best_i)) {
        best = sv[j];
        best_i = si[j];
      }
    unsigned int ub = __float_as_uint(best);
    if ((ub << 1) == 0u) ub = 0u;
    ub = (ub & 0x80000000u) ? ~ub : (ub | 0x80000000u);
    unsigned long long key =
        ((unsigned long long)ub << 32) | (unsigned int)(~best_i);
    atomicMax(Keys + row, key);
  }
}

__global__ void gumbel_unpack_kernel(const unsigned long long* __restrict__ Keys,
                                     int* __restrict__ Out, int rows) {
  int i = blockIdx.x * blockDim.x + threadIdx.x;
  if (i < rows) Out[i] = (int)(~(unsigned int)(Keys[i] & 0xFFFFFFFFull));
}

extern "C" void gumbel_sample(const float* logits, unsigned long long* keys,
                              int* out, int rows, int V, float temperature,
                              unsigned long long seed, hipStream_t stream) {
  const int greedy = temperature > 0.f ? 0 : 1;
  float inv_t = greedy ? 1.f : 1.f / temperature;
  int splits = 1;
  while (rows * splits < 512 && splits * SMP_BLOCK * 4 < V) splits *= 2;
  hipLaunchKernelGGL(gumbel_sample_kernel, dim3(rows * splits),
                     dim3(SMP_BLOCK), 0, stream, logits, keys, rows, V, splits,
                     inv_t, seed, greedy);
  hipLaunchKernelGGL(gumbel_unpack_kernel, dim3((rows + 255) / 256), dim3(256),
                     0, stream, keys, out, rows);
}


__global__ __launch_bounds__(SMP_BLOCK) void softmax_rows_kernel(
    const float* __restrict__ X, float* __restrict__ Y, int rows, int V) {
  int row = blockIdx.x;
  if (row >= rows) return;
  const float* x = X + (long long)row * V;
  float* y = Y + (long long)row * V;
  float m = -1e30f, l = 0.f;
  for (int i = threadIdx.x; i < V; i += SMP_BLOCK) {
    float v = x[i];
    float m_new = fmaxf(m, v);
    l = l * __expf(m - m_new) + __expf(v - m_new);
    m = m_new;
  }
  __shared__ float sm[SMP_BLOCK / WAVE], sl[SMP_BLOCK / WAVE];
#pragma unroll
  for (int s_ = 1; s_ < WAVE; s_ <<= 1) {
    float om = __shfl_xor(m, s_, WAVE);
    float ol = __shfl_xor(l, s_, WAVE);
    float mn = fmaxf(m, om);
    l = l * __expf(m - mn) + ol * __expf(om - mn);
    m = mn;
  }
  int w = threadIdx.x / WAVE;
  if (threadIdx.x % WAVE == 0) {
    sm[w] = m;
    sl[w] = l;
  }
  __syncthreads();
  float M = sm[0], L = sl[0];
  for (int j = 1; j < SMP_BLOCK / WAVE; ++j) {
    float mn = fmaxf(M, sm[j]);
    L = L * __expf(M - mn) + sl[j] * __expf(sm[j] - mn);
    M = mn;
  }
  float inv = 1.f / L;
  for (int i = threadIdx.x; i < V; i += SMP_BLOCK)
    y[i] = __expf(x[i] - M) * inv;
}

extern "C" void softmax_rows(const float* x, float* y, int rows, int V,
                             hipStream_t stream) {
  hipLaunchKernelGGL(softmax_rows_kernel, dim3(rows), dim3(SMP_BLOCK), 0,
                     stream, x, y, rows, V);
}


#define CUT_BLOCK 1024
#define CUT_WAVES (CUT_BLOCK / WAVE)
#define CUT_BINS 4096
#define CUT_PER_THREAD (CUT_BINS / CUT_BLOCK)
#define CUT_NONE 0x7fffffff
#define KEY_NEG_INF 0x007FFFFFu

DEV_INLINE unsigned int fkey(float x) {
  unsigned int u = __float_as_uint(x);
  if ((u << 1) == 0u) u = 0u;
  return (u & 0x80000000u) ? ~u : (u | 0x80000000u);
}

DEV_INLINE float fkey_inv(unsigned int k) {
  return __uint_as_float((k & 0x80000000u) ? (k & 0x7fffffffu) : ~k);
}

DEV_INLINE float row_exp(float x, float inv_t, float m) {
  return expf(__fsub_rn(__fmul_rn(x, inv_t), m));
}

DEV_INLINE unsigned long long mass_fx(float e) {
  return (unsigned long long)(e * 4294967296.f);
}

template <class F>
DEV_INLINE void row_foreach(const float* __restrict__ lg, int V, F f) {
  if ((V & 3) == 0 && ((unsigned long long)lg & 15) == 0) {
    const float4* lg4 = reinterpret_cast<const float4*>(lg);
    const int n4 = V >> 2;
    int i = threadIdx.x;
    for (; i + 3 * CUT_BLOCK < n4; i += 4 * CUT_BLOCK) {
      float4 a = lg4[i], b = lg4[i + CUT_BLOCK], c = lg4[i + 2 * CUT_BLOCK],
             d = lg4[i + 3 * CUT_BLOCK];
      f(a.x); f(a.y); f(a.z); f(a.w);
      f(b.x); f(b.y); f(b.z); f(b.w);
      f(c.x); f(c.y); f(c.z); f(c.w);
      f(d.x); f(d.y); f(d.z); f(d.w);
    }
    for (; i < n4; i += CUT_BLOCK) {
      float4 x = lg4[i];
      f(x.x);
      f(x.y);
      f(x.z);
      f(x.w);
    }
  } else {
    for (int i = threadIdx.x; i < V; i += CUT_BLOCK) f(lg[i]);
  }
}

DEV_INLINE unsigned int block_max_u32(unsigned int v, unsigned int* red) {
#pragma unroll
  for (int s = 1; s < WAVE; s <<= 1) v = max(v, (unsigned int)__shfl_xor((int)v, s, WAVE));
  __syncthreads();
  if (threadIdx.x % WAVE == 0) red[threadIdx.x / WAVE] = v;
  __syncthreads();
  unsigned int r = red[0];
  for (int j = 1; j < CUT_WAVES; ++j) r = max(r, red[j]);
  return r;
}

DEV_INLINE unsigned int block_min_u32(unsigned int v, unsigned int* red) {
  return ~block_max_u32(~v, red);
}

DEV_INLINE int block_sum_i32(int v, unsigned int* red) {
#pragma unroll
  for (int s = 1; s < WAVE; s <<= 1) v += __shfl_xor(v, s, WAVE);
  __syncthreads();
  if (threadIdx.x % WAVE == 0) red[threadIdx.x / WAVE] = (unsigned int)v;
  __syncthreads();
  int r = 0;
  for (int j = 0; j < CUT_WAVES; ++j) r += (int)red[j];
  return r;
}

struct CutShared {
  unsigned long long hist[CUT_BINS];
  unsigned long long wtot[CUT_WAVES];
  unsigned long long sel_above;
  int sel_bin;
  unsigned int red[CUT_WAVES];
};

template <bool MASS>
DEV_INLINE bool radix_select(const float* __restrict__ lg, int V,
                             unsigned int kmin, float inv_t, float m,
                             unsigned long long limit, float p,
                             CutShared& sh, unsigned int* out_key) {
  unsigned int prefix = 0;
  unsigned long long above = 0;
  const int tid = threadIdx.x;
#pragma unroll 1
  for (int level = 0; level < 3; ++level) {
    const int shift = level == 0 ? 20 : level == 1 ? 10 : 0;
    const int bits = level == 0 ? 12 : 10;
    const unsigned int dmask = (1u << bits) - 1u;
    __syncthreads();
#pragma unroll
    for (int j = 0; j < CUT_PER_THREAD; ++j) sh.hist[tid * CUT_PER_THREAD + j] = 0ull;
    if (tid == 0) sh.sel_bin = CUT_NONE;
    __syncthreads();
    row_foreach(lg, V, [&](float x) {
      unsigned int key = fkey(x);
      if (key >= kmin && (level == 0 || ((key >> shift) >> bits) == prefix)) {
        unsigned long long w = MASS ? mass_fx(row_exp(x, inv_t, m)) : 1ull;
        if (w) atomicAdd(&sh.hist[(key >> shift) & dmask], w);
      }
    });
    __syncthreads();
    unsigned long long h[CUT_PER_THREAD];
    unsigned long long ls = 0;
#pragma unroll
    for (int j = 0; j < CUT_PER_THREAD; ++j) {
      h[j] = sh.hist[tid * CUT_PER_THREAD + j];
      ls += h[j];
    }
    unsigned long long incl = ls;
#pragma unroll
    for (int s = 1; s < WAVE; s <<= 1) {
      unsigned long long o = __shfl_up(incl, s, WAVE);
      if ((tid % WAVE) >= s) incl += o;
    }
    if (tid % WAVE == WAVE - 1) sh.wtot[tid / WAVE] = incl;
    __syncthreads();
    unsigned long long total = 0;
    for (int j = 0; j < CUT_WAVES; ++j) {
      if (j < tid / WAVE) incl += sh.wtot[j];
      total += sh.wtot[j];
    }
    if (MASS && level == 0)
      limit = (unsigned long long)((double)p * (double)total);
    unsigned long long u = above + (total - incl);
    int mine = CUT_NONE;
    unsigned long long mine_u = 0;
#pragma unroll
    for (int j = CUT_PER_THREAD - 1; j >= 0; --j) {
      if (h[j] != 0ull && u <= limit) {
        mine = tid * CUT_PER_THREAD + j;
        mine_u = u;
      }
      u += h[j];
    }
    if (mine != CUT_NONE) atomicMin(&sh.sel_bin, mine);
    __syncthreads();
    const int sel = sh.sel_bin;
    if (sel == CUT_NONE) return false;
    if (sel / CUT_PER_THREAD == tid) {
      sh.sel_above = mine_u;
    }
    __syncthreads();
    above = sh.sel_above;
    prefix = (prefix << bits) | (unsigned int)sel;
  }
  *out_key = prefix;
  return true;
}

__global__ __launch_bounds__(CUT_BLOCK) void sampling_cutoff_kernel(
    const float* __restrict__ Logits,
    const float* __restrict__ Temps,
    const int* __restrict__ TopK,
    const float* __restrict__ TopP,
    const float* __restrict__ MinP,
    float* __restrict__ Cut,
    int rows, int V) {
  __shared__ CutShared sh;
  const int row = blockIdx.x;
  if (row >= rows) return;
  const float T = Temps[row];
  const int k = TopK[row];
  const float p = TopP[row];
  const float q = MinP[row];
  const bool k_on = k > 0 && k < V;
  const bool p_on = p < 1.f;
  const bool q_on = q > 0.f;
  const float NEG_INF = __uint_as_float(0xFF800000u);
  if (!(T > 0.f) || !(k_on || p_on || q_on)) {
    if (threadIdx.x == 0) Cut[row] = NEG_INF;
    return;
  }
  const float* lg = Logits + (long long)row * V;
  const float inv_t = 1.f / T;

  unsigned int kmax = 0;
  int nfin = 0;
  row_foreach(lg, V, [&](float x) {
    unsigned int key = fkey(x);
    kmax = max(kmax, key);
    nfin += key > KEY_NEG_INF ? 1 : 0;
  });
  kmax = block_max_u32(kmax, sh.red);
  nfin = block_sum_i32(nfin, sh.red);
  if (nfin == 0 || kmax <= KEY_NEG_INF) {
    if (threadIdx.x == 0) Cut[row] = NEG_INF;
    return;
  }
  const float m = __fmul_rn(fkey_inv(kmax), inv_t);

  unsigned int cut = KEY_NEG_INF + 1u;
  bool ok = true;
  if (k_on) {
    unsigned int kk;
    int keff = min(k, nfin);
    ok = radix_select<false>(lg, V, KEY_NEG_INF + 1u, inv_t, m,
                             (unsigned long long)(keff - 1), 0.f, sh, &kk);
    if (ok) cut = max(cut, kk);
  }
  if (ok && p_on) {
    unsigned int kp;
    ok = radix_select<true>(lg, V, cut, inv_t, m, 0ull, fmaxf(p, 0.f), sh, &kp);
    if (ok) cut = max(cut, kp);
  }
  if (ok && q_on) {
    unsigned int kq = 0xFFFFFFFFu;
    row_foreach(lg, V, [&](float x) {
      unsigned int key = fkey(x);
      if (key > KEY_NEG_INF && row_exp(x, inv_t, m) >= q) kq = min(kq, key);
    });
    kq = block_min_u32(kq, sh.red);
    if (kq != 0xFFFFFFFFu) cut = max(cut, kq);
  }
  if (threadIdx.x == 0) Cut[row] = ok ? fkey_inv(cut) : fkey_inv(kmax);
}

template <bool FILTER>
DEV_INLINE void gumbel_scan(const float* __restrict__ lg, int lo, int hi,
                            float inv_temp, int greedy,
                            unsigned long long seed, unsigned int ctr,
                            float cut, float& best, int& best_i) {
  for (int i = lo + threadIdx.x; i < hi; i += SMP_BLOCK) {
    float x = lg[i];
    float s = x * inv_temp;
    if (!greedy) {
      unsigned int u = hash3((unsigned int)seed, (unsigned int)(seed >> 32) ^ ctr, i);
      float uf = (u >> 8) * (1.f / 16777216.f) + 1e-10f;
      s += -__logf(-__logf(uf));
    }
    if (FILTER) s = x >= cut ? s : __uint_as_float(0xFF800000u);
    if (s > best || (s == best && i < best_i)) {
      best = s;
      best_i = i;
    }
  }
}

__global__ __launch_bounds__(SMP_BLOCK) void gumbel_sample_batch_kernel(
    const float* __restrict__ Logits,
    const float* __restrict__ Temps,
    const long long* __restrict__ Seeds,
    const long long* __restrict__ Counters,
    const float* __restrict__ Cutoff,
    unsigned long long* __restrict__ Keys,
    int rows, int V, int splits) {
  int row = blockIdx.x / splits;
  int split = blockIdx.x % splits;
  if (row >= rows) return;
  const float* lg = Logits + (long long)row * V;
  const float T = Temps[row];
  const int greedy = T > 0.f ? 0 : 1;
  const float inv_temp = greedy ? 1.f : 1.f / T;
  const unsigned long long seed = (unsigned long long)Seeds[row];
  const unsigned int ctr = (unsigned int)(unsigned long long)Counters[row];
  const float NEG_INF = __uint_as_float(0xFF800000u);
  const float cut = (Cutoff != nullptr && !greedy) ? Cutoff[row] : NEG_INF;
  int chunk = (V + splits - 1) / splits;
  int lo = split * chunk, hi = min(V, lo + chunk);
  float best = -1e30f;
  int best_i = lo;
  if (cut == NEG_INF)
    gumbel_scan<false>(lg, lo, hi, inv_temp, greedy, seed, ctr, cut, best, best_i);
  else
    gumbel_scan<true>(lg, lo, hi, inv_temp, greedy, seed, ctr, cut, best, best_i);
#pragma unroll
  for (int s_ = 1; s_ < WAVE; s_ <<= 1) {
    float ov = __shfl_xor(best, s_, WAVE);
    int oi = __shfl_xor(best_i, s_, WAVE);
    if (ov > best || (ov == best && oi < best_i)) {
      best = ov;
      best_i = oi;
    }
  }
  __shared__ float sv[SMP_BLOCK / WAVE];
  __shared__ int si[SMP_BLOCK / WAVE];
  int w = threadIdx.x / WAVE;
  if (threadIdx.x % WAVE == 0) {
    sv[w] = best;
    si[w] = best_i;
  }
  __syncthreads();
  if (threadIdx.x == 0) {
    for (int j = 1; j < SMP_BLOCK / WAVE; ++j)
      if (sv[j] > best || (sv[j] == best && si[j] < best_i)) {
        best = sv[j];
        best_i = si[j];
      }
    unsigned int ub = __float_as_uint(best);
    if ((ub << 1) == 0u) ub = 0u;
    ub = (ub & 0x80000000u) ? ~ub : (ub | 0x80000000u);
    unsigned long long key =
        ((unsigned long long)ub << 32) | (unsigned int)(~best_i);
    atomicMax(Keys + row, key);
  }
}

extern "C" void sampling_cutoff(const float* logits, const float* temps,
                                const int* top_k, const float* top_p,
                                const float* min_p, float* cut, int rows,
                                int V, hipStream_t stream) {
  hipLaunchKernelGGL(sampling_cutoff_kernel, dim3(rows), dim3(CUT_BLOCK), 0,
                     stream, logits, temps, top_k, top_p, min_p, cut, rows, V);
}

extern "C" void gumbel_sample_batch(const float* logits, const float* temps,
                                    const long long* seeds,
                                    const long long* counters,
                                    const float* cutoff,
                                    unsigned long long* keys, int* out,
                                    int rows, int V, hipStream_t stream) {
  int splits = 1;
  while (rows * splits < 512 && splits * SMP_BLOCK * 4 < V) splits *= 2;
  hipLaunchKernelGGL(gumbel_sample_batch_kernel, dim3(rows * splits),
                     dim3(SMP_BLOCK), 0, stream, logits, temps, seeds,
                     counters, cutoff, keys, rows, V, splits);
  hipLaunchKernelGGL(gumbel_unpack_kernel, dim3((rows + 255) / 256), dim3(256),
                     0, stream, keys, out, rows);
}
```

modal_examples_amd/ops/functional.py:

```python
from __future__ import annotations

import math
import os
from typing import Optional

import torch

from . import reference as ref
from ._build import get_ext


def _ext_for(t: torch.Tensor, *grad_tensors, any_dtype: bool = False):
    if torch.is_grad_enabled() and any(
            isinstance(g, torch.Tensor) and g.requires_grad
            for g in (t, *grad_tensors)):
        return None
    if t.is_cuda:
        if not any_dtype and t.dtype is not torch.bfloat16:
            get_ext(required=True)
            return None
        return _sync_wrapped(get_ext(required=True))
    return None


def _sync_wrapped(ext):
    from ..gpu.guard import SyncProxy, debug_sync_enabled

    return SyncProxy(ext) if debug_sync_enabled() else ext


def _attn_train_ext(q, k, v, causal: bool):
    if not (torch.is_grad_enabled()
            and any(t.requires_grad for t in (q, k, v))):
        return None
    if os.environ.get("MODAL_AMD_ATTN_BWD", "") == "ref":
        return None
    if not all(t.is_cuda and t.dtype is torch.bfloat16 for t in (q, k, v)):
        return None
    if q.shape[-1] not in (64, 128) or (causal and q.shape[2] > k.shape[2]):
        return None
    return _sync_wrapped(get_ext(required=True))


def _d_contiguous(t):
    return t if t.stride(-1) == 1 else t.contiguous()


class _AttentionFn(torch.autograd.Function):

    @staticmethod
    def forward(ctx, q, k, v, causal, scale, bshd, ext):
        q, k, v = _d_contiguous(q), _d_contiguous(k), _d_contiguous(v)
        if bshd:
            o, lse = ext.attention_fwd_lse_bshd(q, k, v, causal, scale)
        else:
            o, lse = ext.attention_fwd_lse(q, k, v, causal, scale)
        ctx.save_for_backward(q, k, v, o, lse)
        ctx.causal, ctx.scale, ctx.bshd, ctx.ext = causal, scale, bshd, ext
        return o

    @staticmethod
    @torch.autograd.function.once_differentiable
    def backward(ctx, dout):
        q, k, v, o, lse = ctx.saved_tensors
        if ctx.bshd:
            o, dout = o.transpose(1, 2), dout.transpose(1, 2)
        dout = _d_contiguous(dout)

        def grad_like(t):
            if ctx.bshd:
                B, H, S, D = t.shape
                return torch.empty(B, S, H, D, dtype=t.dtype,
                                   device=t.device).transpose(1, 2)
            return torch.empty(t.shape, dtype=t.dtype, device=t.device)

        dq, dk, dv = grad_like(q), grad_like(k), grad_like(v)
        ctx.ext.attention_bwd(q, k, v, o, lse, dout, dq, dk, dv, ctx.causal,
                              ctx.scale)
        return dq, dk, dv, None, None, None, None


def _attention(q, k, v, causal, scale, bshd: bool):
    scale = scale if scale is not None else 1.0 / math.sqrt(q.shape[-1])
    if k.shape[2] == 0:
        raise ValueError("attention: Sk must be at least 1, got Sk=0 (a query "
                         "with no key has no softmax)")
    ext = _attn_train_ext(q, k, v, causal)
    if ext is not None:
        return _AttentionFn.apply(q, k, v, causal, scale, bshd, ext)
    ext = _ext_for(q, k, v)
    if ext is None:
        o = ref.attention_ref(q, k, v, causal, scale)
        return o.transpose(1, 2) if bshd else o
    if bshd:
        return ext.attention_bshd(q, k, v, causal, scale)
    return ext.attention(q.contiguous(), k.contiguous(), v.contiguous(),
                         causal, scale)


def attention(q, k, v, causal: bool = False, scale: Optional[float] = None):
    return _attention(q, k, v, causal, scale, False)


def attention_qkv(q, k, v, causal: bool = False, scale: Optional[float] = None):
    B, S, Hq, D = q.shape
    o = _attention(q.transpose(1, 2), k.transpose(1, 2), v.transpose(1, 2),
                   causal, scale, True)
    return o.reshape(B, S, Hq * D)


def paged_decode(q, k_cache, v_cache, block_table, seq_lens, block_size: int = 0,
                 scale: Optional[float] = None):
    scale = scale if scale is not None else 1.0 / math.sqrt(q.shape[-1])
    ext = _ext_for(q)
    if ext is None:
        if k_cache.dtype not in (torch.float32, torch.bfloat16, torch.float16):
            k_cache = k_cache.to(torch.float32)
            v_cache = v_cache.to(torch.float32)
        return ref.paged_decode_ref(q, k_cache, v_cache, block_table, seq_lens,
                                    block_size, scale)
    bt = block_table.contiguous() if block_table is not None else None
    return ext.paged_decode(q.contiguous(), k_cache, v_cache, bt,
                            seq_lens.int(), block_size, scale)


def paged_prefill(q, k_cache, v_cache, block_table, cu_q, seq_lens,
                  block_size: int, scale: Optional[float] = None,
                  max_q_len: Optional[int] = None):
    if block_table is None:
        raise ValueError("paged_prefill needs a block_table (there is no "
                         "contiguous-cache mode)")
    scale = scale if scale is not None else 1.0 / math.sqrt(q.shape[-1])
    ext = _ext_for(q)
    if ext is None:
        if k_cache.dtype not in (torch.float32, torch.float64, torch.bfloat16,
                                 torch.float16):
            k_cache = k_cache.to(torch.float32)
            v_cache = v_cache.to(torch.float32)
        return ref.paged_prefill_ref(q, k_cache, v_cache, block_table, cu_q,
                                     seq_lens, block_size, scale)
    return ext.paged_prefill(q.contiguous(), k_cache, v_cache,
                             block_table.contiguous(), cu_q.int().contiguous(),
                             seq_lens.int().contiguous(), block_size, scale,
                             q.shape[0] if max_q_len is None else max_q_len)


def groupnorm_silu(x, gamma, beta, groups: int = 32, eps: float = 1e-5,
                   do_silu: bool = True):
    ext = _ext_for(x, gamma, beta)
    if ext is None:
        return ref.groupnorm_silu_ref(x, gamma, beta, groups, eps, do_silu)
    return ext.groupnorm_silu(x.contiguous(), gamma.float().contiguous(),
                              beta.float().contiguous(), groups, eps, do_silu)


def layernorm(x, gamma, beta, eps: float = 1e-5):
    ext = _ext_for(x, gamma, beta)
    if ext is None:
        return ref.layernorm_ref(x, gamma, beta, eps)
    return ext.layernorm(x.contiguous(), gamma.float().contiguous(),
                         beta.float().contiguous(), eps)


def rmsnorm(x, gamma, eps: float = 1e-6):
    ext = _ext_for(x, gamma)
    if ext is None:
        return ref.rmsnorm_ref(x, gamma, eps)
    return ext.rmsnorm(x.contiguous(), gamma.float().contiguous(), eps)


def cfg_euler(x_t, eps_c, eps_u, guidance: float, dsigma: float):
    ext = _ext_for(x_t)
    if ext is None:
        return ref.cfg_euler_ref(x_t, eps_c, eps_u, guidance, dsigma)
    return ext.cfg_euler(x_t.contiguous(), eps_c.contiguous(),
                         eps_u.contiguous() if eps_u is not None else None,
                         guidance, dsigma)


def silu_mul(a, b):
    ext = _ext_for(a, b)
    if ext is None:
        return ref.silu_mul_ref(a, b)
    return ext.silu_mul(a.contiguous(), b.contiguous())


def geglu(a, b):
    ext = _ext_for(a, b)
    if ext is None:
        return ref.geglu_ref(a, b)
    return ext.geglu(a.contiguous(), b.contiguous())


def glu_fused(src, gelu: bool = False):
    inner = src.shape[-1] // 2
    ext = _ext_for(src)
    if ext is None or inner % 8 != 0:
        a, b = src[..., :inner], src[..., inner:]
        return (ref.geglu_ref(a, b) if gelu else ref.silu_mul_ref(a, b))
    return ext.glu_fused(src.contiguous(), gelu)


def add_residual(a, b):
    ext = _ext_for(a, b)
    if ext is None:
        return (a.float() + b.float()).to(a.dtype)
    return ext.add_residual(a.contiguous(), b.contiguous())


def rope(x, cos, sin, positions=None, inplace: bool = False):
    ext = _ext_for(x)
    if ext is None:
        if positions is not None and positions.numel() == x.shape[0] * x.shape[2] \
                and x.shape[0] > 1:
            B, H, S, D = x.shape
            pos = positions.view(B, S).long()
            outs = [ref.rope_ref(x[b:b + 1], cos, sin, pos[b]) for b in range(B)]
            return torch.cat(outs, 0)
        return ref.rope_ref(x, cos, sin, positions.long() if positions is not None else None)
    assert x.stride(-1) == 1, "rope needs contiguous head_dim"
    y = x if inplace else x.clone()
    pos = positions
    if pos is not None:
        pos = pos.int()
        if pos.numel() == x.shape[2] and x.shape[0] > 1:
            pos = pos.repeat(x.shape[0])
    ext.rope_(y, cos.float().contiguous(), sin.float().contiguous(), pos)
    return y


def rope_tables(max_seq: int, dim: int, base: float = 10000.0, device="cpu"):
    inv = 1.0 / (base ** (torch.arange(0, dim, 2, dtype=torch.float64) / dim))
    t = torch.arange(max_seq, dtype=torch.float64)
    freqs = torch.outer(t, inv)
    return (freqs.cos().float().to(device), freqs.sin().float().to(device))


def repack_conv3x3_weight(weight: torch.Tensor) -> torch.Tensor:
    K, C = weight.shape[0], weight.shape[1]
    kpad = (K + 63) // 64 * 64
    c16 = (C + 15) // 16 * 16
    wr = torch.zeros(9, kpad, c16, dtype=torch.bfloat16, device=weight.device)
    w = weight.permute(2, 3, 0, 1).reshape(9, K, C)
    wr[:, :K, :C] = w.to(torch.bfloat16)
    return wr.contiguous()


def conv3x3(x, wr, bias, K: int, residual=None, raw_weight=None,
            upsample: bool = False):
    ext = _ext_for(x, raw_weight if raw_weight is not None else x)
    if ext is None:
        assert raw_weight is not None, "reference conv path needs raw_weight"
        xin = x
        if upsample:
            xin = torch.nn.functional.interpolate(x, scale_factor=2.0,
                                                  mode="nearest")
        y = torch.nn.functional.conv2d(
            xin.float(), raw_weight.float(), bias.float(), padding=1)
        if residual is not None:
            y = y + residual.float()
        return y.to(x.dtype)
    out = ext.conv3x3(x.contiguous(), wr, bias,
                      residual.contiguous() if residual is not None else None,
                      K, upsample)
    return out


def conv3x3_gn(x, wr, bias, K: int, gamma, beta, groups: int = 32,
               eps: float = 1e-5, residual=None, raw_weight=None,
               upsample: bool = False):
    ext = _ext_for(x, raw_weight if raw_weight is not None else x)
    if ext is None:
        assert raw_weight is not None
        h = torch.nn.functional.group_norm(x.float(), groups, gamma.float(),
                                           beta.float(), eps)
        h = torch.nn.functional.silu(h)
        if upsample:
            h = torch.nn.functional.interpolate(h, scale_factor=2.0,
                                                mode="nearest")
        y = torch.nn.functional.conv2d(h, raw_weight.float(), bias.float(),
                                       padding=1)
        if residual is not None:
            y = y + residual.float()
        return y.to(x.dtype)
    return ext.conv3x3_gn(x.contiguous(), wr, bias,
                          residual.contiguous() if residual is not None else None,
                          K, upsample, gamma.float().contiguous(),
                          beta.float().contiguous(), groups, eps)


def adamw_step(p, g, m, v, lr, beta1=0.9, beta2=0.999, eps=1e-8, wd=0.01, step=1):
    ext = _ext_for(p, any_dtype=True)
    if ext is None:
        return ref.adamw_ref(p, g, m, v, lr, beta1, beta2, eps, wd, step)
    ext.adamw_(p, g.contiguous(), m, v, lr, beta1, beta2, eps, wd, step)
    return p


def sample(logits, temperature: float = 1.0, seed: int = 0):
    ext = _ext_for(logits, any_dtype=True)
    if ext is None:
        if temperature <= 0:
            return logits.argmax(-1).int()
        g = torch.Generator(device="cpu").manual_seed(seed or 1)
        u = torch.rand(logits.shape, generator=g).clamp_min(1e-10)
        gumbel = -(-u.log()).log()
        return (logits.float() / temperature + gumbel).argmax(-1).int()
    return ext.sample_gumbel(logits.float().contiguous(), temperature, seed)


def wrap_int64(v: int) -> int:
    v = int(v) & (1 << 64) - 1
    return v - (1 << 64) if v >= 1 << 63 else v


def _row_param(v, rows: int, dtype, device, name: str) -> torch.Tensor:
    if isinstance(v, torch.Tensor):
        if v.dim() == 0:
            v = v.expand(rows)
        if v.dim() != 1 or v.shape[0] != rows:
            raise ValueError(f"{name} must have one value per row ([{rows}]), "
                             f"got {tuple(v.shape)}")
        if v.device != device:
            raise ValueError(f"{name} is on {v.device}, logits on {device}")
        return v.to(dtype).contiguous()
    if dtype is torch.int64:
        v = wrap_int64(v)
    return torch.full((rows,), v, dtype=dtype, device=device)


def _check_logits_2d(logits):
    if logits.dim() != 2 or logits.shape[0] == 0 or logits.shape[1] == 0:
        raise ValueError(f"logits must be [rows, V], got {tuple(logits.shape)}")


def _filter_params(logits, temperature, top_k, top_p, min_p):
    rows, dev = logits.shape[0], logits.device
    return (_row_param(temperature, rows, torch.float32, dev, "temperature"),
            _row_param(0 if top_k is None else top_k, rows, torch.int32, dev,
                       "top_k"),
            _row_param(1.0 if top_p is None else top_p, rows, torch.float32,
                       dev, "top_p"),
            _row_param(0.0 if min_p is None else min_p, rows, torch.float32,
                       dev, "min_p"))


def sampling_cutoff(logits, temperature, top_k=None, top_p=None, min_p=None):
    _check_logits_2d(logits)
    t, k, p, q = _filter_params(logits, temperature, top_k, top_p, min_p)
    ext = _ext_for(logits, any_dtype=True)
    if ext is None:
        return ref.sampling_cutoff_ref(logits, t, k, p, q)
    return ext.sampling_cutoff(logits.float().contiguous(), t, k, p, q)


def sample_batch(logits, temperature, top_k=None, top_p=None, min_p=None,
                 seeds=None, counters=None):
    _check_logits_2d(logits)
    rows, dev = logits.shape[0], logits.device
    s = _row_param(0 if seeds is None else seeds, rows, torch.int64, dev,
                   "seeds")
    c = (torch.arange(rows, dtype=torch.int64, device=dev) if counters is None
         else _row_param(counters, rows, torch.int64, dev, "counters"))
    ext = _ext_for(logits, any_dtype=True)
    if ext is None:
        t, k, p, q = _filter_params(logits, temperature, top_k, top_p, min_p)
        return ref.sample_batch_ref(logits, t, k, p, q, s, c)
    lg = logits.float().contiguous()
    if top_k is None and top_p is None and min_p is None:
        t = _row_param(temperature, rows, torch.float32, dev, "temperature")
        return ext.sample_batch(lg, t, s, c, None)
    t, k, p, q = _filter_params(logits, temperature, top_k, top_p, min_p)
    return ext.sample_batch(lg, t, s, c, ext.sampling_cutoff(lg, t, k, p, q))


def softmax(x):
    ext = _ext_for(x, any_dtype=True)
    if ext is None:
        return torch.softmax(x.float(), dim=-1)
    return ext.softmax_fwd(x.float().contiguous())



def _check_moe_route(logits, top_k):
    if logits.dim() != 2 or logits.shape[0] < 1:
        raise ValueError(f"logits must be [N, E] with N >= 1, got "
                         f"{tuple(logits.shape)}")
    E = logits.shape[1]
    if not 1 <= E <= 128:
        raise ValueError(f"logits has E={E} experts (supported: 1..128)")
    if not isinstance(top_k, int) or not 1 <= top_k <= min(E, 8):
        raise ValueError(f"top_k={top_k!r} (supported: 1..min(E, 8) = "
                         f"{min(E, 8)})")


def moe_route(logits, top_k: int):
    _check_moe_route(logits, top_k)
    ext = _ext_for(logits, any_dtype=True)
    if ext is None:
        return ref.moe_route_ref(logits, top_k)
    return ext.moe_route(logits.float().contiguous(), top_k)


def _check_moe_ffn(x, gate_up, down, weights, idx):
    if x.dim() != 2 or x.shape[0] < 1:
        raise ValueError(f"x must be [N, dim] with N >= 1, got "
                         f"{tuple(x.shape)}")
    N, d = x.shape
    if d % 64 != 0:
        raise ValueError(f"x has dim={d} (must be a multiple of 64)")
    if gate_up.dim() != 3 or gate_up.shape[2] != d \
            or gate_up.shape[1] % 2 != 0:
        raise ValueError(f"gate_up must be [E, 2*ffn_dim, dim={d}], got "
                         f"{tuple(gate_up.shape)}")
    E, F = gate_up.shape[0], gate_up.shape[1] // 2
    if not 1 <= E <= 128:
        raise ValueError(f"gate_up has E={E} experts (supported: 1..128)")
    if F % 64 != 0 or F < 64:
        raise ValueError(f"gate_up has ffn_dim={F} (must be a multiple of "
                         f"64)")
    if tuple(down.shape) != (E, d, F):
        raise ValueError(f"down must be [E={E}, dim={d}, ffn_dim={F}], got "
                         f"{tuple(down.shape)}")
    if idx.dtype is not torch.int32:
        raise TypeError(f"idx must be int32, got {idx.dtype}")
    if idx.dim() != 2 or idx.shape[0] != N \
            or not 1 <= idx.shape[1] <= min(E, 8):
        raise ValueError(f"idx must be [N={N}, top_k] with top_k in "
                         f"1..min(E, 8) = {min(E, 8)}, got {tuple(idx.shape)}")
    if weights.shape != idx.shape:
        raise ValueError(f"weights must have idx's shape "
                         f"{tuple(idx.shape)}, got {tuple(weights.shape)}")
    for name, t in (("x", x), ("gate_up", gate_up), ("down", down)):
        if not t.is_contiguous():
            raise ValueError(f"{name} must be contiguous")
        if t.dtype is not x.dtype or t.device != x.device:
            raise ValueError(f"{name} must have x's dtype and device "
                             f"({x.dtype}, {x.device}), got {t.dtype}, "
                             f"{t.device}")


def moe_ffn(x, gate_up, down, weights, idx):
    _check_moe_ffn(x, gate_up, down, weights, idx)
    ext = _ext_for(x, gate_up, down, weights)
    if ext is None:
        return ref.moe_ffn_ref(x, gate_up, down, weights, idx)
    return ext.moe_ffn(x, gate_up, down, weights.float().contiguous(),
                       idx.contiguous())
```

Before: 19.63 images/s.

## Fuse residual adds, layout transposes, and timestep addend into SDXL custom kernels

Adds several fused HIP kernels to the SDXL UNet and VAE. They cover GroupNorm+SiLU writing NHWC output directly, an add+LayerNorm that produces both the residual sum and its normalization, an NHWC-to-NCHW residual add using an LDS transpose, a scaled bf16 softmax, and a per-[N,K] addend folded into the conv3x3 epilogue for the timestep embedding. These remove separate elementwise kernels, permute/contiguous copies and fp32 softmax round trips. The cost is more custom code paths, with small numeric differences from rounding the scaled scores to bf16.

```diff
diff --git a/modal_examples_amd/models/sdxl/layers.py b/modal_examples_amd/models/sdxl/layers.py
--- a/modal_examples_amd/models/sdxl/layers.py
+++ b/modal_examples_amd/models/sdxl/layers.py
@@ -55,9 +55,10 @@
         self.eps = eps
         self.silu = silu
 
-    def forward(self, x):
+    def forward(self, x, out_nhwc: bool = False):
         return OF.groupnorm_silu(x, self._f32("weight"), self._f32("bias"),
-                                 self.groups, self.eps, self.silu)
+                                 self.groups, self.eps, self.silu,
+                                 out_nhwc=out_nhwc)
 
 
 class Conv3x3(nn.Conv2d):
@@ -95,14 +96,17 @@
                                  raw_weight=self.weight, upsample=upsample)
         return self.forward(gn(x), residual=residual, upsample=upsample)
 
-    def forward(self, x, residual=None, upsample: bool = False):
+    def forward(self, x, residual=None, upsample: bool = False, addend=None):
         if self._use_kernel(x):
             wr, b = self._packed()
             return OF.conv3x3(x, wr, b, self.out_channels, residual=residual,
-                              raw_weight=self.weight, upsample=upsample)
+                              raw_weight=self.weight, upsample=upsample,
+                              addend=addend)
         if upsample:
             x = nn.functional.interpolate(x, scale_factor=2.0, mode="nearest")
         y = nn.functional.conv2d(x, self.weight, self.bias, padding=1)
+        if addend is not None:
+            y = y + addend[:, :, None, None]
         return y if residual is None else y + residual
 
 
@@ -173,10 +177,12 @@
         self.ff = GEGLUFeedForward(dim)
 
     def forward(self, x, ctx):
-        x = x + self.attn1(self.norm1(x))
-        x = x + self.attn2(self.norm2(x), ctx)
-        x = x + self.ff(self.norm3(x))
-        return x
+        n2, n3 = self.norm2, self.norm3
+        x, h = OF.add_layernorm(x, self.attn1(self.norm1(x)),
+                                n2._f32("weight"), n2._f32("bias"), n2.eps)
+        x, h = OF.add_layernorm(x, self.attn2(h, ctx),
+                                n3._f32("weight"), n3._f32("bias"), n3.eps)
+        return x + self.ff(h)
 
 
 def timestep_embedding(t: torch.Tensor, dim: int, max_period: float = 10000.0):
diff --git a/modal_examples_amd/models/sdxl/unet.py b/modal_examples_amd/models/sdxl/unet.py
--- a/modal_examples_amd/models/sdxl/unet.py
+++ b/modal_examples_amd/models/sdxl/unet.py
@@ -5,6 +5,7 @@
 import torch
 import torch.nn as nn
 
+from ...ops import functional as OF
 from .layers import (
     Conv1x1,
     Conv3x3,
@@ -51,8 +52,8 @@
         self.skip = Conv1x1(c_in, c_out) if c_in != c_out else nn.Identity()
 
     def forward(self, x, temb):
-        h = self.conv1(self.norm1(x))
-        h = h + self.temb_proj(torch.nn.functional.silu(temb))[:, :, None, None]
+        t = self.temb_proj(torch.nn.functional.silu(temb))
+        h = self.conv1(self.norm1(x), addend=t)
         return self.conv2(self.norm2(h), residual=self.skip(x))
 
 
@@ -68,14 +69,10 @@
         self.proj_out = nn.Linear(channels, channels)
 
     def forward(self, x, ctx):
-        B, C, H, W = x.shape
-        res = x
-        h = self.norm(x).permute(0, 2, 3, 1).reshape(B, H * W, C)
-        h = self.proj_in(h)
+        h = self.proj_in(self.norm(x, out_nhwc=True))
         for blk in self.blocks:
             h = blk(h, ctx)
-        h = self.proj_out(h)
-        return res + h.reshape(B, H, W, C).permute(0, 3, 1, 2)
+        return OF.add_nhwc_to_nchw(x, self.proj_out(h))
 
 
 class Downsample(nn.Module):
diff --git a/modal_examples_amd/models/sdxl/vae.py b/modal_examples_amd/models/sdxl/vae.py
--- a/modal_examples_amd/models/sdxl/vae.py
+++ b/modal_examples_amd/models/sdxl/vae.py
@@ -3,6 +3,7 @@
 import torch
 import torch.nn as nn
 
+from ...ops import functional as OF
 from .layers import Conv1x1, Conv3x3, GroupNormSiLU
 
 
@@ -33,16 +34,14 @@
         self.scale = c ** -0.5
 
     def forward(self, x):
-        B, C, H, W = x.shape
-        h = self.norm(x).permute(0, 2, 3, 1).reshape(B, H * W, C)
+        h = self.norm(x, out_nhwc=True)
         q, k, v = self.q(h), self.k(h), self.v(h)
         outs = []
         for i in range(0, q.shape[1], self.chunk):
-            s = torch.matmul(q[:, i:i + self.chunk], k.transpose(1, 2)) * self.scale
-            p = torch.softmax(s.float(), dim=-1).to(v.dtype)
-            outs.append(torch.matmul(p, v))
+            s = torch.matmul(q[:, i:i + self.chunk], k.transpose(1, 2))
+            outs.append(torch.matmul(OF.scaled_softmax(s, self.scale), v))
         o = self.out(torch.cat(outs, dim=1))
-        return x + o.reshape(B, H, W, C).permute(0, 3, 1, 2)
+        return OF.add_nhwc_to_nchw(x, o)
 
 
 class VAEDecoder(nn.Module):
diff --git a/modal_examples_amd/ops/csrc/bindings.cpp b/modal_examples_amd/ops/csrc/bindings.cpp
--- a/modal_examples_amd/ops/csrc/bindings.cpp
+++ b/modal_examples_amd/ops/csrc/bindings.cpp
@@ -22,8 +22,17 @@
 void groupnorm_silu_bf16(const void*, void*, float*, const float*,
                          const float*, int, int, long long, int, float, int,
                          hipStream_t);
+void groupnorm_silu_nhwc_bf16(const void*, void*, float*, const float*,
+                              const float*, int, int, long long, int, float,
+                              int, hipStream_t);
 void layernorm_bf16(const void*, void*, const float*, const float*, long long,
                     int, float, hipStream_t);
+void add_layernorm_bf16(const void*, const void*, void*, void*, const float*,
+                        const float*, long long, int, float, hipStream_t);
+void add_nhwc_to_nchw_bf16(const void*, const void*, void*, int, int,
+                           long long, hipStream_t);
+void scaled_softmax_bf16(const void*, void*, long long, int, float,
+                         hipStream_t);
 void rmsnorm_bf16(const void*, void*, const float*, long long, int, float,
                   hipStream_t);
 void cfg_euler_bf16(const void*, const void*, const void*, void*, float, float,
@@ -51,9 +60,9 @@
                         const float*, const long long*, float, long long,
                         hipStream_t);
 void advance_step(long long*, hipStream_t);
-void conv3x3_bf16(const void*, const void*, const void*, const void*, void*,
-                  const float*, const float*, int, int, int, int, int, int,
-                  int, int, hipStream_t);
+void conv3x3_bf16(const void*, const void*, const void*, const void*,
+                  const void*, void*, const float*, const float*, int, int,
+                  int, int, int, int, int, int, hipStream_t);
 void gn_conv_coeffs_bf16(const void*, float*, const float*, const float*,
                          float*, float*, int, int, int, long long, int, float,
                          hipStream_t);
@@ -365,6 +374,77 @@
   return y;
 }
 
+void check_f32_param(const char* op, const torch::Tensor& t, const char* name,
+                     int64_t n) {
+  TORCH_CHECK(t.is_cuda(), op, ": ", name, " must be on GPU");
+  TORCH_CHECK(t.scalar_type() == torch::kFloat, op, ": ", name,
+              " must be fp32");
+  TORCH_CHECK(t.is_contiguous() && t.dim() == 1 && t.numel() == n, op, ": ",
+              name, " must be a contiguous vector of ", n, " elements, got ",
+              t.sizes());
+}
+
+void check_same_device(const char* op, const torch::Tensor& a,
+                       const torch::Tensor& b, const char* name) {
+  TORCH_CHECK(a.device() == b.device(), op, ": ", name, " is on ", b.device(),
+              ", expected ", a.device());
+}
+
+torch::Tensor groupnorm_silu_nhwc(torch::Tensor x, torch::Tensor gamma,
+                                  torch::Tensor beta, int64_t groups,
+                                  double eps, bool do_silu) {
+  const char* op = "groupnorm_silu_nhwc";
+  check_bf16(x, "x");
+  TORCH_CHECK(x.dim() == 4, op, ": x must be NCHW, got ", x.dim(), " dims");
+  const int64_t N = x.size(0), C = x.size(1), HW = x.size(2) * x.size(3);
+  TORCH_CHECK(groups >= 1 && C >= 1 && C % groups == 0, op,
+              ": groups must be at least 1 and divide C, got groups=", groups,
+              " C=", C);
+  check_f32_param(op, gamma, "gamma", C);
+  check_f32_param(op, beta, "beta", C);
+  check_same_device(op, x, gamma, "gamma");
+  check_same_device(op, x, beta, "beta");
+  TORCH_CHECK(N <= 65535 && HW < (1ll << 31) && C < (1ll << 22) &&
+                  N * groups < (1ll << 20),
+              op, ": too large for the kernel (N <= 65535, H*W < 2^31, "
+              "C < 2^22, N*groups < 2^20), got x ", x.sizes());
+  auto y = torch::empty({N, HW, C}, x.options());
+  auto ws = torch::zeros({N * groups * 2}, x.options().dtype(torch::kFloat32));
+  groupnorm_silu_nhwc_bf16(x.data_ptr(), y.data_ptr(), ws.data_ptr<float>(),
+                           gamma.data_ptr<float>(), beta.data_ptr<float>(),
+                           (int)N, (int)C, HW, (int)groups, (float)eps,
+                           do_silu ? 1 : 0, cur_stream());
+  return y;
+}
+
+std::vector<torch::Tensor> add_layernorm(torch::Tensor x, torch::Tensor y,
+                                         torch::Tensor gamma,
+                                         torch::Tensor beta, double eps) {
+  const char* op = "add_layernorm";
+  check_bf16(x, "x");
+  check_bf16(y, "y");
+  check_same_device(op, x, y, "y");
+  TORCH_CHECK(x.dim() >= 1 && x.sizes() == y.sizes(), op,
+              ": x and y must have one shape, got ", x.sizes(), " and ",
+              y.sizes());
+  const int64_t D = x.size(-1);
+  TORCH_CHECK(D >= 8 && D % 8 == 0 && D < (1ll << 31), op,
+              ": the last dimension must be a positive multiple of 8 (rows "
+              "start on 16-byte boundaries), got ", D);
+  check_f32_param(op, gamma, "gamma", D);
+  check_f32_param(op, beta, "beta", D);
+  check_same_device(op, x, gamma, "gamma");
+  check_same_device(op, x, beta, "beta");
+  const int64_t rows = x.numel() / D;
+  TORCH_CHECK((rows + 3) / 4 < (1ll << 31), op, ": too many rows: ", rows);
+  auto s = torch::empty_like(x);
+  auto ln = torch::empty_like(x);
+  add_layernorm_bf16(x.data_ptr(), y.data_ptr(), s.data_ptr(), ln.data_ptr(),
+                     gamma.data_ptr<float>(), beta.data_ptr<float>(), rows,
+                     (int)D, (float)eps, cur_stream());
+  return {s, ln};
+}
+
 torch::Tensor rmsnorm(torch::Tensor x, torch::Tensor gamma, double eps) {
   check_bf16(x, "x");
   int D = x.size(-1);
@@ -422,6 +502,44 @@
   check_bf16(a, "a");
   auto y = torch::empty_like(a);
   add_bf16(a.data_ptr(), b.data_ptr(), y.data_ptr(), a.numel(), cur_stream());
+  return y;
+}
+
+torch::Tensor add_nhwc_to_nchw(torch::Tensor res, torch::Tensor h) {
+  const char* op = "add_nhwc_to_nchw";
+  check_bf16(res, "res");
+  check_bf16(h, "h");
+  check_same_device(op, res, h, "h");
+  TORCH_CHECK(res.dim() == 4, op, ": res must be NCHW, got ", res.dim(),
+              " dims");
+  const int64_t N = res.size(0), C = res.size(1),
+                HW = res.size(2) * res.size(3);
+  TORCH_CHECK(h.dim() == 3 && h.size(0) == N && h.size(1) == HW &&
+                  h.size(2) == C,
+              op, ": h must be [N, H*W, C] = [", N, ", ", HW, ", ", C,
+              "], got ", h.sizes());
+  TORCH_CHECK(N <= 65535 && HW < (1ll << 31) && C < (1ll << 22), op,
+              ": too large for the kernel (N <= 65535, H*W < 2^31, C < 2^22), "
+              "got res ", res.sizes());
+  auto out = torch::empty_like(res);
+  add_nhwc_to_nchw_bf16(res.data_ptr(), h.data_ptr(), out.data_ptr(), (int)N,
+                        (int)C, HW, cur_stream());
+  return out;
+}
+
+torch::Tensor scaled_softmax(torch::Tensor s, double scale) {
+  const char* op = "scaled_softmax";
+  check_bf16(s, "s");
+  TORCH_CHECK(s.dim() >= 1, op, ": s must have at least one dimension");
+  const int64_t V = s.size(-1);
+  TORCH_CHECK(V >= 8 && V % 8 == 0 && V < (1ll << 31), op,
+              ": the last dimension must be a positive multiple of 8, got ",
+              V);
+  const int64_t rows = s.numel() / V;
+  TORCH_CHECK(rows < (1ll << 31), op, ": too many rows: ", rows);
+  auto y = torch::empty_like(s);
+  scaled_softmax_bf16(s.data_ptr(), y.data_ptr(), rows, (int)V, (float)scale,
+                      cur_stream());
   return y;
 }
 
@@ -506,11 +624,23 @@
 
 torch::Tensor conv3x3(torch::Tensor x, torch::Tensor wr, torch::Tensor bias,
                       c10::optional<torch::Tensor> residual, int64_t K,
-                      bool upsample) {
+                      bool upsample, c10::optional<torch::Tensor> addend) {
   const ConvDims d = check_conv("conv3x3", x, wr, bias, residual, K, upsample);
+  if (addend.has_value()) {
+    TORCH_CHECK(!residual.has_value(),
+                "conv3x3: addend and residual cannot be combined");
+    check_bf16(*addend, "addend");
+    TORCH_CHECK(addend->device() == x.device(), "conv3x3: addend is on ",
+                addend->device(), ", x on ", x.device());
+    TORCH_CHECK(addend->dim() == 2 && addend->size(0) == d.N &&
+                    addend->size(1) == K,
+                "conv3x3: addend must be [N, K] = [", d.N, ", ", K, "], got ",
+                addend->sizes());
+  }
   auto out = torch::empty({d.N, K, d.Ho, d.Wo}, x.options());
   conv3x3_bf16(x.data_ptr(), wr.data_ptr(), bias.data_ptr(),
                residual.has_value() ? residual->data_ptr() : nullptr,
+               addend.has_value() ? addend->data_ptr() : nullptr,
                out.data_ptr(), nullptr, nullptr, d.N, d.C, d.Ho, d.Wo, (int)K,
                d.C16, d.Kpad, upsample ? 1 : 0, cur_stream());
   return out;
@@ -540,7 +670,7 @@
   auto out = torch::empty({N, K, d.Ho, d.Wo}, x.options());
   conv3x3_bf16(x.data_ptr(), wr.data_ptr(), bias.data_ptr(),
                residual.has_value() ? residual->data_ptr() : nullptr,
-               out.data_ptr(), scale.data_ptr<float>(),
+               nullptr, out.data_ptr(), scale.data_ptr<float>(),
                shift.data_ptr<float>(), N, d.C, d.Ho, d.Wo, (int)K, C16,
                d.Kpad, upsample ? 1 : 0, cur_stream());
   return out;
@@ -805,7 +935,15 @@
         "paged KV prefill attention: ragged causal chunks over a cached "
         "prefix (K6)");
   m.def("groupnorm_silu", &groupnorm_silu);
+  m.def("groupnorm_silu_nhwc", &groupnorm_silu_nhwc,
+        "GroupNorm(+SiLU) of NCHW x, written as [N, H*W, C]");
   m.def("layernorm", &layernorm);
+  m.def("add_layernorm", &add_layernorm,
+        "(x + y, LayerNorm(x + y)) from one read of x and y");
+  m.def("add_nhwc_to_nchw", &add_nhwc_to_nchw,
+        "res [N,C,H,W] + h [N,H*W,C], tiled transpose in LDS");
+  m.def("scaled_softmax", &scaled_softmax,
+        "softmax((s * scale).float(), -1).to(bf16), bf16 in and out");
   m.def("rmsnorm", &rmsnorm);
   m.def("cfg_euler", &cfg_euler, "fused CFG + Euler step (K4)");
   m.def("silu_mul", &silu_mul);
@@ -819,7 +957,12 @@
         "per-row temperature/seed/counter/cutoff gumbel sampling (K8)");
   m.def("sampling_cutoff", &sampling_cutoff_fwd,
         "per-row top-k/top-p/min-p logit cutoff by radix select (K8)");
-  m.def("conv3x3", &conv3x3, "NCHW implicit-GEMM 3x3 conv, fused bias+res (K3)");
+  m.def("conv3x3", &conv3x3,
+        "NCHW implicit-GEMM 3x3 conv, fused bias + residual or [N,K] addend "
+        "(K3)",
+        pybind11::arg("x"), pybind11::arg("wr"), pybind11::arg("bias"),
+        pybind11::arg("residual"), pybind11::arg("K"),
+        pybind11::arg("upsample"), pybind11::arg("addend") = pybind11::none());
   m.def("conv3x3_gn", &conv3x3_gn, "GroupNorm+SiLU fused into the K3 conv");
   m.def("softmax_fwd", &softmax_fwd);
   m.def("moe_route", &moe_route,
diff --git a/modal_examples_amd/ops/csrc/conv3x3.hip b/modal_examples_amd/ops/csrc/conv3x3.hip
--- a/modal_examples_amd/ops/csrc/conv3x3.hip
+++ b/modal_examples_amd/ops/csrc/conv3x3.hip
@@ -34,7 +34,7 @@
 void conv3x3_kernel(
     const short* __restrict__ in, const short* __restrict__ wr,
     const float* __restrict__ bias, const short* __restrict__ res,
-    short* __restrict__ out, const float* __restrict__ gn_scale,
+    const short* __restrict__ addend, short* __restrict__ out, const float* __restrict__ gn_scale,
     const float* __restrict__ gn_shift, int C, int H, int W, int Hs, int Ws,
     int K, int C16, int Kpad, int npix_x, int npix, int nk) {
   constexpr int CV_ROWS = CV_NW * RPW;
@@ -46,6 +46,7 @@
   __shared__ alignas(16) short patch[PATCH_ELEMS];
   __shared__ alignas(16) short wlds[WLDS_ELEMS];
   __shared__ alignas(16) float bias_s[CV_BK];
+  __shared__ alignas(16) float addend_s[CV_BK];
 
   const int tid = threadIdx.x;
   const int w = tid / WAVE;
@@ -71,7 +72,11 @@
   const long long in_n = (long long)n * C * Hs * Ws;
   const int nc = C16 / CV_CC;
 
-  if (tid < CV_BK) bias_s[tid] = bias[min(k0 + tid, K - 1)];
+  if (tid < CV_BK) {
+    const int kc = min(k0 + tid, K - 1);
+    bias_s[tid] = bias[kc];
+    if (addend != nullptr) addend_s[tid] = bf2f(addend[(long long)n * K + kc]);
+  }
 
   const char* in_img = (const char*)(in + in_n);
   const unsigned hwb = (unsigned)Hs * (unsigned)Ws * 2u;
@@ -222,8 +227,9 @@
     }
   }
 
-  auto epilogue = [&](auto res_c, auto edge_c) {
+  auto epilogue = [&](auto res_c, auto add_c, auto edge_c) {
     constexpr bool RES = decltype(res_c)::value;
+    constexpr bool ADD = decltype(add_c)::value;
     constexpr bool EDGE = decltype(edge_c)::value;
     int t = tid;
     asm volatile("" : "+v"(t));
@@ -254,12 +260,16 @@
 #pragma unroll
         for (int q = 0; q < 4; ++q) {
           const f32x4 b4 = *(const f32x4*)&bias_s[mf * 32 + 8 * q + 4 * hi5];
+          f32x4 a4;
+          if constexpr (ADD)
+            a4 = *(const f32x4*)&addend_s[mf * 32 + 8 * q + 4 * hi5];
 #pragma unroll
           for (int j = 0; j < 4; ++j) {
             const int r = q * 4 + j;
             const int kl = mf * 32 + j + 8 * q + 4 * hi5;
             float v = acc[rr][mf][r] + b4[j];
             if constexpr (RES) v += bf2f((short)rv[r]);
+            if constexpr (ADD) v = bf2f(f2bf(v)) + a4[j];
             if (!EDGE || (pix_ok && kl <= kmax))
               *(short*)(outb + (po + (unsigned)kl * hw) * 2u) = f2bf(v);
           }
@@ -269,17 +279,23 @@
   };
   const bool edge =
       y0 + CV_ROWS > H || x0 + CV_COLS > W || k0 + CV_BK > K;
+  const std::true_type yes{};
+  const std::false_type no{};
   if (res != nullptr) {
-    if (edge) epilogue(std::true_type{}, std::true_type{});
-    else epilogue(std::true_type{}, std::false_type{});
+    if (edge) epilogue(yes, no, yes);
+    else epilogue(yes, no, no);
+  } else if (addend != nullptr) {
+    if (edge) epilogue(no, yes, yes);
+    else epilogue(no, yes, no);
   } else {
-    if (edge) epilogue(std::false_type{}, std::true_type{});
-    else epilogue(std::false_type{}, std::false_type{});
+    if (edge) epilogue(no, no, yes);
+    else epilogue(no, no, no);
   }
 }
 
 extern "C" void conv3x3_bf16(const void* in, const void* wrepack,
-                             const void* bias, const void* residual, void* out,
+                             const void* bias, const void* residual,
+                             const void* addend, void* out,
                              const float* gn_scale, const float* gn_shift,
                              int N, int C, int H, int W, int K, int C16,
                              int Kpad, int upsample, hipStream_t stream) {
@@ -300,7 +316,8 @@
 #define CVL(UPV, GNV, RPWV) \
   hipLaunchKernelGGL((conv3x3_kernel<UPV, GNV, RPWV>), grid, block, 0, \
                      stream, (const short*)in, (const short*)wrepack, \
-                     (const float*)bias, (const short*)residual, (short*)out, \
+                     (const float*)bias, (const short*)residual, \
+                     (const short*)addend, (short*)out, \
                      gn_scale, gn_shift, C, H, W, Hs, Ws, K, C16, Kpad, \
                      npix_x, npix, nk)
   if (rpw == 4) {
diff --git a/modal_examples_amd/ops/csrc/elementwise.hip b/modal_examples_amd/ops/csrc/elementwise.hip
--- a/modal_examples_amd/ops/csrc/elementwise.hip
+++ b/modal_examples_amd/ops/csrc/elementwise.hip
@@ -140,6 +140,87 @@
   int grid = elementwise_grid(n, EW_BLOCK);
   hipLaunchKernelGGL(add_kernel, dim3(grid), dim3(EW_BLOCK), 0, stream,
                      (const short*)a, (const short*)b, (short*)y, n);
+}
+
+#define AT 64
+#define AT_LD (AT + 2)
+
+__global__ __launch_bounds__(256) void add_nhwc_to_nchw_kernel(
+    const short* __restrict__ R, const short* __restrict__ Hh,
+    short* __restrict__ O, int C, int HW) {
+  __shared__ alignas(16) unsigned tile[AT * AT_LD / 2];
+  const int n = blockIdx.z;
+  const int c0 = blockIdx.y * AT, p0 = blockIdx.x * AT;
+  const int lane = threadIdx.x % WAVE, wv = threadIdx.x / WAVE;
+  const int ca = c0 + 2 * (lane % 8 + 8 * wv);
+  const int pl = (lane / 8) * 8, pa = p0 + pl;
+  short rv[2][8];
+#pragma unroll
+  for (int h = 0; h < 2; ++h) {
+    const int c = ca + h;
+    const short* rr = R + ((long long)n * C + c) * HW;
+    if (c < C && (HW % 8) == 0 && pa < HW) {
+      const bf16x8 t = *(const bf16x8*)&rr[pa];
+#pragma unroll
+      for (int j = 0; j < 8; ++j) rv[h][j] = t[j];
+    } else {
+#pragma unroll
+      for (int j = 0; j < 8; ++j)
+        rv[h][j] = (c < C && pa + j < HW) ? rr[pa + j] : (short)0;
+    }
+  }
+#pragma unroll
+  for (int i = 0; i < 2; ++i) {
+    const int pr = threadIdx.x / 8 + 32 * i, pb = p0 + pr;
+    const int cl = (threadIdx.x % 8) * 8, cb = c0 + cl;
+    unsigned d[4] = {0u, 0u, 0u, 0u};
+    if (pb < HW && cb < C) {
+      const short* hr = Hh + ((long long)n * HW + pb) * C;
+      if ((C % 8) == 0) {
+        const i32x4 t = *(const i32x4*)&hr[cb];
+#pragma unroll
+        for (int q = 0; q < 4; ++q) d[q] = (unsigned)t[q];
+      } else {
+#pragma unroll
+        for (int j = 0; j < 8; ++j)
+          if (cb + j < C)
+            d[j / 2] |= (unsigned)(unsigned short)hr[cb + j] << (16 * (j & 1));
+      }
+    }
+#pragma unroll
+    for (int q = 0; q < 4; ++q) tile[(pr * AT_LD + cl) / 2 + q] = d[q];
+  }
+  __syncthreads();
+  bf16x8 o[2];
+#pragma unroll
+  for (int j = 0; j < 8; ++j) {
+    const unsigned t = tile[((pl + j) * AT_LD + (ca - c0)) / 2];
+    o[0][j] = f2bf(bf2f(rv[0][j]) + bf2f((short)(t & 0xffffu)));
+    o[1][j] = f2bf(bf2f(rv[1][j]) + bf2f((short)(t >> 16)));
+  }
+#pragma unroll
+  for (int h = 0; h < 2; ++h) {
+    const int c = ca + h;
+    short* orow = O + ((long long)n * C + c) * HW;
+    if (c >= C || pa >= HW) continue;
+    if ((HW % 8) == 0) {
+      *(bf16x8*)&orow[pa] = o[h];
+    } else {
+#pragma unroll
+      for (int j = 0; j < 8; ++j)
+        if (pa + j < HW) orow[pa + j] = o[h][j];
+    }
+  }
+}
+
+extern "C" void add_nhwc_to_nchw_bf16(const void* res, const void* h,
+                                      void* out, int N, int C, long long HW,
+                                      hipStream_t stream) {
+  if (N == 0 || C == 0 || HW == 0) return;
+  dim3 grid((unsigned)((HW + AT - 1) / AT), (C + AT - 1) / AT, N);
+  hipLaunchKernelGGL(add_nhwc_to_nchw_kernel, grid, dim3(256), 0, stream,
+                     (const short*)res, (const short*)h, (short*)out, C,
+                     (int)HW);
 }
 
 
diff --git a/modal_examples_amd/ops/csrc/norms.hip b/modal_examples_amd/ops/csrc/norms.hip
--- a/modal_examples_amd/ops/csrc/norms.hip
+++ b/modal_examples_amd/ops/csrc/norms.hip
@@ -43,6 +43,25 @@
   }
 }
 
+DEV_INLINE void gn_stats(const float* __restrict__ WS, int ng, float slab,
+                         float eps, float& mean, float& rstd) {
+  mean = WS[ng * 2] / slab;
+  const float var = fmaf(-mean, mean, WS[ng * 2 + 1] / slab);
+  rstd = rsqrtf(var + eps);
+}
+
+DEV_INLINE void gn_coeff(float gamma_c, float beta_c, float mean, float rstd,
+                         float& gam, float& bet) {
+  gam = gamma_c * rstd;
+  bet = fmaf(-mean, gam, beta_c);
+}
+
+DEV_INLINE float gn_elem(short x, float gam, float bet, int do_silu) {
+  float f = fmaf(bf2f(x), gam, bet);
+  if (do_silu) f = f / (1.f + __expf(-f));
+  return f;
+}
+
 __global__ __launch_bounds__(256) void gn_norm_kernel(
     const short* __restrict__ X, short* __restrict__ Y,
     const float* __restrict__ WS, const float* __restrict__ gamma,
@@ -56,38 +75,120 @@
   const long long slab = (long long)cpg * HW;
   const short* x = X + ((long long)n * C + (long long)g * cpg) * HW;
   short* y = Y + ((long long)n * C + (long long)g * cpg) * HW;
-  float mean = WS[ng * 2] / (float)slab;
-  float var = WS[ng * 2 + 1] / (float)slab - mean * mean;
-  float rstd = rsqrtf(var + eps);
+  float mean, rstd;
+  gn_stats(WS, ng, (float)slab, eps, mean, rstd);
   long long per = (((HW + split - 1) / split) + 7) & ~7LL;
   long long lo = sp * per, hi = min(HW, lo + per);
   if (lo >= HW) return;
   for (int c = 0; c < cpg; ++c) {
     const short* xc = x + (long long)c * HW;
     short* yc = y + (long long)c * HW;
-    float gam = gamma[g * cpg + c] * rstd;
-    float bet = beta[g * cpg + c] - mean * gam;
+    float gam, bet;
+    gn_coeff(gamma[g * cpg + c], beta[g * cpg + c], mean, rstd, gam, bet);
     long long i = lo + (long long)threadIdx.x * 8;
     for (; i + 8 <= hi; i += 256 * 8) {
       bf16x8 v = *(const bf16x8*)&xc[i];
       bf16x8 o;
 #pragma unroll
-      for (int j = 0; j < 8; ++j) {
-        float f = bf2f(v[j]) * gam + bet;
-        if (do_silu) f = f / (1.f + __expf(-f));
-        o[j] = f2bf(f);
-      }
+      for (int j = 0; j < 8; ++j) o[j] = f2bf(gn_elem(v[j], gam, bet, do_silu));
       *(bf16x8*)&yc[i] = o;
     }
     long long tail = hi - ((hi - lo) % 8);
     for (long long t = tail + threadIdx.x; t < hi; t += 256) {
-      if (t >= lo) {
-        float f = bf2f(xc[t]) * gam + bet;
-        if (do_silu) f = f / (1.f + __expf(-f));
-        yc[t] = f2bf(f);
+      if (t >= lo) yc[t] = f2bf(gn_elem(xc[t], gam, bet, do_silu));
+    }
+  }
+}
+
+#define TT 64
+#define TT_LD (TT + 2)
+
+__global__ __launch_bounds__(256) void gn_norm_nhwc_kernel(
+    const short* __restrict__ X, short* __restrict__ Y,
+    const float* __restrict__ WS, const float* __restrict__ gamma,
+    const float* __restrict__ beta, int C, int HW, int G, float eps,
+    int do_silu) {
+  __shared__ alignas(16) unsigned tile[TT * TT_LD / 2];
+  const int n = blockIdx.z;
+  const int c0 = blockIdx.y * TT, p0 = blockIdx.x * TT;
+  const int cpg = C / G;
+  const int lane = threadIdx.x % WAVE, wv = threadIdx.x / WAVE;
+  {
+    const int ca = c0 + 2 * (lane % 8 + 8 * wv);
+    const int pl = (lane / 8) * 8, pa = p0 + pl;
+    short v[2][8];
+#pragma unroll
+    for (int h = 0; h < 2; ++h) {
+      const int c = ca + h;
+      const short* xr = X + ((long long)n * C + c) * HW;
+      if (c < C && (HW % 8) == 0 && pa < HW) {
+        const bf16x8 t = *(const bf16x8*)&xr[pa];
+#pragma unroll
+        for (int j = 0; j < 8; ++j) v[h][j] = t[j];
+      } else {
+#pragma unroll
+        for (int j = 0; j < 8; ++j)
+          v[h][j] = (c < C && pa + j < HW) ? xr[pa + j] : (short)0;
       }
     }
-  }
+    float gam[2], bet[2];
+#pragma unroll
+    for (int h = 0; h < 2; ++h) {
+      const int c = min(ca + h, C - 1);
+      float mean, rstd;
+      gn_stats(WS, n * G + c / cpg, (float)((long long)cpg * HW), eps, mean,
+               rstd);
+      gn_coeff(gamma[c], beta[c], mean, rstd, gam[h], bet[h]);
+    }
+#pragma unroll
+    for (int j = 0; j < 8; ++j) {
+      const unsigned lo =
+          (unsigned short)f2bf(gn_elem(v[0][j], gam[0], bet[0], do_silu));
+      const unsigned hi =
+          (unsigned short)f2bf(gn_elem(v[1][j], gam[1], bet[1], do_silu));
+      tile[((pl + j) * TT_LD + (ca - c0)) / 2] = lo | (hi << 16);
+    }
+  }
+  __syncthreads();
+#pragma unroll
+  for (int i = 0; i < 2; ++i) {
+    const int pr = threadIdx.x / 8 + 32 * i, pb = p0 + pr;
+    const int cl = (threadIdx.x % 8) * 8, cb = c0 + cl;
+    if (pb >= HW || cb >= C) continue;
+    unsigned d[4];
+#pragma unroll
+    for (int q = 0; q < 4; ++q) d[q] = tile[(pr * TT_LD + cl) / 2 + q];
+    short* yr = Y + ((long long)n * HW + pb) * C;
+    if ((C % 8) == 0) {
+      i32x4 o = {(int)d[0], (int)d[1], (int)d[2], (int)d[3]};
+      *(i32x4*)&yr[cb] = o;
+    } else {
+#pragma unroll
+      for (int j = 0; j < 8; ++j)
+        if (cb + j < C) yr[cb + j] = (short)(d[j / 2] >> (16 * (j & 1)));
+    }
+  }
+}
+
+static int gn_split(int N, int G, long long HW) {
+  int split = 1;
+  while (N * G * split < 1024 && (long long)split * 2048 < HW) split *= 2;
+  return split;
+}
+
+extern "C" void groupnorm_silu_nhwc_bf16(const void* x, void* y, float* ws,
+                                         const float* gamma, const float* beta,
+                                         int N, int C, long long HW, int G,
+                                         float eps, int do_silu,
+                                         hipStream_t stream) {
+  if (N == 0 || C == 0 || HW == 0) return;
+  const int split = gn_split(N, G, HW);
+  hipLaunchKernelGGL(gn_partial_kernel, dim3(N * G * split), dim3(256), 0,
+                     stream, (const short*)x, ws, N, C, HW, G, split);
+  dim3 grid((unsigned)((HW + TT - 1) / TT), (C + TT - 1) / TT, N);
+  hipLaunchKernelGGL(gn_norm_nhwc_kernel, grid, dim3(256), 0, stream,
+                     (const short*)x, (short*)y, ws, gamma, beta, C, (int)HW,
+                     G, eps, do_silu);
 }
 
 extern "C" void groupnorm_silu_bf16(const void* x, void* y, float* ws,
@@ -95,8 +196,7 @@
                                     int N, int C, long long HW, int G,
                                     float eps, int do_silu,
                                     hipStream_t stream) {
-  int split = 1;
-  while (N * G * split < 1024 && (long long)split * 2048 < HW) split *= 2;
+  const int split = gn_split(N, G, HW);
   dim3 grid(N * G * split);
   hipLaunchKernelGGL(gn_partial_kernel, grid, dim3(256), 0, stream,
                      (const short*)x, ws, N, C, HW, G, split);
@@ -105,6 +205,84 @@
                      eps, do_silu, split);
 }
 
+
+struct LnSrcPlain {
+  const short* x;
+  DEV_INLINE bf16x8 vec(int i, bool) const { return *(const bf16x8*)&x[i]; }
+  DEV_INLINE short one(int i, bool) const { return x[i]; }
+};
+
+struct LnSrcAdd {
+  const short* x;
+  const short* y;
+  short* s;
+  DEV_INLINE bf16x8 vec(int i, bool first) const {
+    const bf16x8 a = *(const bf16x8*)&x[i];
+    const bf16x8 b = *(const bf16x8*)&y[i];
+    bf16x8 o;
+#pragma unroll
+    for (int j = 0; j < 8; ++j) o[j] = f2bf(bf2f(a[j]) + bf2f(b[j]));
+    if (first) *(bf16x8*)&s[i] = o;
+    return o;
+  }
+  DEV_INLINE short one(int i, bool first) const {
+    const short o = f2bf(bf2f(x[i]) + bf2f(y[i]));
+    if (first) s[i] = o;
+    return o;
+  }
+};
+
+template <int NV, class Src>
+DEV_INLINE void ln_row(const Src& src, short* __restrict__ y,
+                       const float* __restrict__ gamma,
+                       const float* __restrict__ beta, int D, float eps,
+                       int l) {
+  bf16x8 keep[NV > 0 ? NV : 1];
+  float s = 0.f, ss = 0.f;
+  auto stat = [&](const bf16x8& v) {
+#pragma unroll
+    for (int j = 0; j < 8; ++j) {
+      float f = bf2f(v[j]);
+      s += f;
+      ss += f * f;
+    }
+  };
+#pragma unroll
+  for (int k = 0; k < NV; ++k) {
+    const int i = l * 8 + k * WAVE * 8;
+    if (i + 8 <= D) {
+      keep[k] = src.vec(i, true);
+      stat(keep[k]);
+    }
+  }
+  for (int i = l * 8 + NV * WAVE * 8; i + 8 <= D; i += WAVE * 8)
+    stat(src.vec(i, true));
+  for (int i = (D / 8) * 8 + l; i < D; i += WAVE) {
+    float f = bf2f(src.one(i, true));
+    s += f;
+    ss += f * f;
+  }
+  s = wave_sum(s);
+  ss = wave_sum(ss);
+  float mean = s / D, var = ss / D - mean * mean;
+  float rstd = rsqrtf(var + eps);
+  auto norm = [&](const bf16x8& v, int i) {
+    bf16x8 o;
+#pragma unroll
+    for (int j = 0; j < 8; ++j)
+      o[j] = f2bf((bf2f(v[j]) - mean) * rstd * gamma[i + j] + beta[i + j]);
+    *(bf16x8*)&y[i] = o;
+  };
+#pragma unroll
+  for (int k = 0; k < NV; ++k) {
+    const int i = l * 8 + k * WAVE * 8;
+    if (i + 8 <= D) norm(keep[k], i);
+  }
+  for (int i = l * 8 + NV * WAVE * 8; i + 8 <= D; i += WAVE * 8)
+    norm(src.vec(i, false), i);
+  for (int i = (D / 8) * 8 + l; i < D; i += WAVE)
+    y[i] = f2bf((bf2f(src.one(i, false)) - mean) * rstd * gamma[i] + beta[i]);
+}
 
 __global__ __launch_bounds__(256) void layernorm_kernel(
     const short* __restrict__ X, short* __restrict__ Y,
@@ -113,37 +291,7 @@
   int w = threadIdx.x / WAVE, l = threadIdx.x % WAVE;
   long long row = (long long)blockIdx.x * 4 + w;
   if (row >= rows) return;
-  const short* x = X + row * D;
-  short* y = Y + row * D;
-  float s = 0.f, ss = 0.f;
-  for (int i = l * 8; i + 8 <= D; i += WAVE * 8) {
-    bf16x8 v = *(const bf16x8*)&x[i];
-#pragma unroll
-    for (int j = 0; j < 8; ++j) {
-      float f = bf2f(v[j]);
-      s += f;
-      ss += f * f;
-    }
-  }
-  for (int i = (D / 8) * 8 + l; i < D; i += WAVE) {
-    float f = bf2f(x[i]);
-    s += f;
-    ss += f * f;
-  }
-  s = wave_sum(s);
-  ss = wave_sum(ss);
-  float mean = s / D, var = ss / D - mean * mean;
-  float rstd = rsqrtf(var + eps);
-  for (int i = l * 8; i + 8 <= D; i += WAVE * 8) {
-    bf16x8 v = *(const bf16x8*)&x[i];
-    bf16x8 o;
-#pragma unroll
-    for (int j = 0; j < 8; ++j)
-      o[j] = f2bf((bf2f(v[j]) - mean) * rstd * gamma[i + j] + beta[i + j]);
-    *(bf16x8*)&y[i] = o;
-  }
-  for (int i = (D / 8) * 8 + l; i < D; i += WAVE)
-    y[i] = f2bf((bf2f(x[i]) - mean) * rstd * gamma[i] + beta[i]);
+  ln_row<0>(LnSrcPlain{X + row * D}, Y + row * D, gamma, beta, D, eps, l);
 }
 
 extern "C" void layernorm_bf16(const void* x, void* y, const float* gamma,
@@ -153,6 +301,38 @@
   hipLaunchKernelGGL(layernorm_kernel, dim3((unsigned)blocks), dim3(256), 0,
                      stream, (const short*)x, (short*)y, gamma, beta, rows, D,
                      eps);
+}
+
+
+template <int NV>
+__global__ __launch_bounds__(256) void add_layernorm_kernel(
+    const short* __restrict__ X, const short* __restrict__ Yin,
+    short* __restrict__ S, short* __restrict__ LN,
+    const float* __restrict__ gamma, const float* __restrict__ beta,
+    long long rows, int D, float eps) {
+  int w = threadIdx.x / WAVE, l = threadIdx.x % WAVE;
+  long long row = (long long)blockIdx.x * 4 + w;
+  if (row >= rows) return;
+  ln_row<NV>(LnSrcAdd{X + row * D, Yin + row * D, S + row * D}, LN + row * D,
+             gamma, beta, D, eps, l);
+}
+
+extern "C" void add_layernorm_bf16(const void* x, const void* y, void* s,
+                                   void* ln, const float* gamma,
+                                   const float* beta, long long rows, int D,
+                                   float eps, hipStream_t stream) {
+  if (rows == 0 || D == 0) return;
+  long long blocks = (rows + 3) / 4;
+  const int nv = (D / 8 + WAVE - 1) / WAVE;
+#define ALN(NVV) \
+  hipLaunchKernelGGL(add_layernorm_kernel<NVV>, dim3((unsigned)blocks), \
+                     dim3(256), 0, stream, (const short*)x, (const short*)y, \
+                     (short*)s, (short*)ln, gamma, beta, rows, D, eps)
+  if (nv <= 1) ALN(1);
+  else if (nv <= 2) ALN(2);
+  else if (nv <= 3) ALN(3);
+  else ALN(4);
+#undef ALN
 }
 
 
@@ -222,8 +402,7 @@
                                     float* scale, float* shift, int N, int C,
                                     int Cpad, long long HW, int G, float eps,
                                     hipStream_t stream) {
-  int split = 1;
-  while (N * G * split < 1024 && (long long)split * 2048 < HW) split *= 2;
+  const int split = gn_split(N, G, HW);
   hipLaunchKernelGGL(gn_partial_kernel, dim3(N * G * split), dim3(256), 0,
                      stream, (const short*)x, ws, N, C, HW, G, split);
   hipLaunchKernelGGL(gn_coeff_kernel, dim3((N * Cpad + 255) / 256), dim3(256),
diff --git a/modal_examples_amd/ops/csrc/sampling.hip b/modal_examples_amd/ops/csrc/sampling.hip
--- a/modal_examples_amd/ops/csrc/sampling.hip
+++ b/modal_examples_amd/ops/csrc/sampling.hip
@@ -133,6 +133,135 @@
                              hipStream_t stream) {
   hipLaunchKernelGGL(softmax_rows_kernel, dim3(rows), dim3(SMP_BLOCK), 0,
                      stream, x, y, rows, V);
+}
+
+
+#define SSM_MAX_NV 8
+
+DEV_INLINE float ssm_block_max(float v, float* sh) {
+  v = wave_max(v);
+  const int w = threadIdx.x / WAVE;
+  if (threadIdx.x % WAVE == 0) sh[w] = v;
+  __syncthreads();
+  float r = sh[0];
+#pragma unroll
+  for (int j = 1; j < SMP_BLOCK / WAVE; ++j) r = fmaxf(r, sh[j]);
+  return r;
+}
+
+DEV_INLINE float ssm_block_sum(float v, float* sh) {
+  v = wave_sum(v);
+  const int w = threadIdx.x / WAVE;
+  if (threadIdx.x % WAVE == 0) sh[w] = v;
+  __syncthreads();
+  float r = sh[0];
+#pragma unroll
+  for (int j = 1; j < SMP_BLOCK / WAVE; ++j) r += sh[j];
+  return r;
+}
+
+DEV_INLINE float ssm_scaled(short s, float scale) {
+  return bf2f(f2bf(bf2f(s) * scale));
+}
+
+template <int NV>
+__global__ __launch_bounds__(SMP_BLOCK) void scaled_softmax_kernel(
+    const short* __restrict__ X, short* __restrict__ Y, int V, float scale) {
+  __shared__ float shm[SMP_BLOCK / WAVE], shs[SMP_BLOCK / WAVE];
+  const long long row = blockIdx.x;
+  const short* x = X + row * V;
+  short* y = Y + row * V;
+  const int nvec = V / 8;
+  float f[NV][8];
+  float m = -INFINITY;
+#pragma unroll
+  for (int k = 0; k < NV; ++k) {
+    const int vi = k * SMP_BLOCK + threadIdx.x;
+    if (vi < nvec) {
+      const bf16x8 v = *(const bf16x8*)&x[vi * 8];
+#pragma unroll
+      for (int j = 0; j < 8; ++j) {
+        f[k][j] = ssm_scaled(v[j], scale);
+        m = fmaxf(m, f[k][j]);
+      }
+    }
+  }
+  m = ssm_block_max(m, shm);
+  float l = 0.f;
+#pragma unroll
+  for (int k = 0; k < NV; ++k) {
+    const int vi = k * SMP_BLOCK + threadIdx.x;
+    if (vi < nvec) {
+#pragma unroll
+      for (int j = 0; j < 8; ++j) {
+        f[k][j] = __expf(f[k][j] - m);
+        l += f[k][j];
+      }
+    }
+  }
+  l = ssm_block_sum(l, shs);
+  const float inv = 1.f / l;
+#pragma unroll
+  for (int k = 0; k < NV; ++k) {
+    const int vi = k * SMP_BLOCK + threadIdx.x;
+    if (vi < nvec) {
+      bf16x8 o;
+#pragma unroll
+      for (int j = 0; j < 8; ++j) o[j] = f2bf(f[k][j] * inv);
+      *(bf16x8*)&y[vi * 8] = o;
+    }
+  }
+}
+
+__global__ __launch_bounds__(SMP_BLOCK) void scaled_softmax_long_kernel(
+    const short* __restrict__ X, short* __restrict__ Y, int V, float scale) {
+  __shared__ float shm[SMP_BLOCK / WAVE], shs[SMP_BLOCK / WAVE];
+  const long long row = blockIdx.x;
+  const short* x = X + row * V;
+  short* y = Y + row * V;
+  const int nvec = V / 8;
+  float m = -INFINITY;
+  for (int vi = threadIdx.x; vi < nvec; vi += SMP_BLOCK) {
+    const bf16x8 v = *(const bf16x8*)&x[vi * 8];
+#pragma unroll
+    for (int j = 0; j < 8; ++j) m = fmaxf(m, ssm_scaled(v[j], scale));
+  }
+  m = ssm_block_max(m, shm);
+  float l = 0.f;
+  for (int vi = threadIdx.x; vi < nvec; vi += SMP_BLOCK) {
+    const bf16x8 v = *(const bf16x8*)&x[vi * 8];
+#pragma unroll
+    for (int j = 0; j < 8; ++j) l += __expf(ssm_scaled(v[j], scale) - m);
+  }
+  l = ssm_block_sum(l, shs);
+  const float inv = 1.f / l;
+  for (int vi = threadIdx.x; vi < nvec; vi += SMP_BLOCK) {
+    const bf16x8 v = *(const bf16x8*)&x[vi * 8];
+    bf16x8 o;
+#pragma unroll
+    for (int j = 0; j < 8; ++j)
+      o[j] = f2bf(__expf(ssm_scaled(v[j], scale) - m) * inv);
+    *(bf16x8*)&y[vi * 8] = o;
+  }
+}
+
+extern "C" void scaled_softmax_bf16(const void* x, void* y, long long rows,
+                                    int V, float scale, hipStream_t stream) {
+  if (rows == 0 || V == 0) return;
+  const int nv = (V / 8 + SMP_BLOCK - 1) / SMP_BLOCK;
+#define SSM(NVV) \
+  hipLaunchKernelGGL(scaled_softmax_kernel<NVV>, dim3((unsigned)rows), \
+                     dim3(SMP_BLOCK), 0, stream, (const short*)x, (short*)y, \
+                     V, scale)
+  if (nv <= 1) SSM(1);
+  else if (nv <= 2) SSM(2);
+  else if (nv <= 4) SSM(4);
+  else if (nv <= SSM_MAX_NV) SSM(SSM_MAX_NV);
+  else
+    hipLaunchKernelGGL(scaled_softmax_long_kernel, dim3((unsigned)rows),
+                       dim3(SMP_BLOCK), 0, stream, (const short*)x, (short*)y,
+                       V, scale);
+#undef SSM
 }
 
 
diff --git a/modal_examples_amd/ops/functional.py b/modal_examples_amd/ops/functional.py
--- a/modal_examples_amd/ops/functional.py
+++ b/modal_examples_amd/ops/functional.py
@@ -146,12 +146,17 @@
 
 
 def groupnorm_silu(x, gamma, beta, groups: int = 32, eps: float = 1e-5,
-                   do_silu: bool = True):
+                   do_silu: bool = True, out_nhwc: bool = False):
     ext = _ext_for(x, gamma, beta)
     if ext is None:
-        return ref.groupnorm_silu_ref(x, gamma, beta, groups, eps, do_silu)
-    return ext.groupnorm_silu(x.contiguous(), gamma.float().contiguous(),
-                              beta.float().contiguous(), groups, eps, do_silu)
+        y = ref.groupnorm_silu_ref(x, gamma, beta, groups, eps, do_silu)
+        if out_nhwc:
+            N, C, H, W = x.shape
+            y = y.permute(0, 2, 3, 1).reshape(N, H * W, C)
+        return y
+    fn = ext.groupnorm_silu_nhwc if out_nhwc else ext.groupnorm_silu
+    return fn(x.contiguous(), gamma.float().contiguous(),
+              beta.float().contiguous(), groups, eps, do_silu)
 
 
 def layernorm(x, gamma, beta, eps: float = 1e-5):
@@ -160,6 +165,34 @@
         return ref.layernorm_ref(x, gamma, beta, eps)
     return ext.layernorm(x.contiguous(), gamma.float().contiguous(),
                          beta.float().contiguous(), eps)
+
+
+def add_layernorm(x, y, gamma, beta, eps: float = 1e-5):
+    ext = _ext_for(x, y, gamma, beta)
+    if ext is None or x.shape[-1] % 8 != 0 or x.shape != y.shape \
+            or y.dtype is not x.dtype:
+        s = x + y
+        return s, layernorm(s, gamma, beta, eps)
+    s, ln = ext.add_layernorm(x.contiguous(), y.contiguous(),
+                              gamma.float().contiguous(),
+                              beta.float().contiguous(), eps)
+    return s, ln
+
+
+def add_nhwc_to_nchw(res, h):
+    N, C, H, W = res.shape
+    ext = _ext_for(res, h)
+    if ext is None or h.dtype is not res.dtype:
+        return res + h.reshape(N, H, W, C).permute(0, 3, 1, 2)
+    return ext.add_nhwc_to_nchw(res.contiguous(), h.contiguous())
+
+
+def scaled_softmax(s, scale: float):
+    ext = _ext_for(s)
+    if ext is None or s.shape[-1] % 8 != 0 or s.shape[-1] == 0 \
+            or not s.is_contiguous():
+        return torch.softmax((s * scale).float(), dim=-1).to(s.dtype)
+    return ext.scaled_softmax(s, scale)
 
 
 def rmsnorm(x, gamma, eps: float = 1e-6):
@@ -247,8 +280,16 @@
 
 
 def conv3x3(x, wr, bias, K: int, residual=None, raw_weight=None,
-            upsample: bool = False):
-    ext = _ext_for(x, raw_weight if raw_weight is not None else x)
+            upsample: bool = False, addend=None):
+    if addend is not None and residual is not None:
+        raise ValueError("conv3x3: addend and residual cannot be combined")
+    ext = _ext_for(x, raw_weight if raw_weight is not None else x, addend)
+    if ext is not None and addend is not None:
+        return ext.conv3x3(x.contiguous(), wr, bias, None, K, upsample,
+                           addend.contiguous())
+    if addend is not None:
+        return conv3x3(x, wr, bias, K, raw_weight=raw_weight,
+                       upsample=upsample) + addend[:, :, None, None]
     if ext is None:
         assert raw_weight is not None, "reference conv path needs raw_weight"
         xin = x
```

After: 20.60 images/s, median of 6. +4.9%, better.
